# Kangfei/NNGP-src

Hardware: AMD Instinct MI355X
Metric: NNGP kernel-build + GP-solve wall-clock (ms) and GFLOP/s at N train queries (higher is better)
Workload: dtype f32 (Cholesky products as split f16 x3, f32 accumulate; f64 build/CG/means; the posterior's float64-grade residual as exact int8 digit-plane products); 1 GPU; synthetic N=32768, d=128, 5-layer ReLU NNGP + full Cholesky posterior (configs[2], north-star target); N=32768, d=128, n_relu=3, get=nngp, M_test=1024, parallelism=single GPU

## Files before the change

__graft_entry__.py:

```python
import os
import subprocess
import sys

ROOT = os.path.dirname(os.path.abspath(__file__))
for _p in (ROOT, os.path.join(ROOT, "oracle")):
    if _p not in sys.path:
        sys.path.insert(0, _p)


def build() -> None:
    env = dict(os.environ)
    env.setdefault("HIPCC", "/opt/rocm/bin/hipcc")
    subprocess.check_call(["make", "-C", os.path.join(ROOT, "nngp-src_amd", "csrc"), "-j8", "ARCH=gfx950"], env=env)
    subprocess.check_call(["make", "-C", os.path.join(ROOT, "oracle")])
    import nngp_src_amd
    from nngp_src_amd import _lib
    lib = _lib.load()
    assert lib.nngp_version() == 1
    for name in _lib.ABI_SYMBOLS + _lib.GP_ABI_SYMBOLS + _lib.ACT_ABI_SYMBOLS + _lib.MLL_ABI_SYMBOLS + _lib.LOO_ABI_SYMBOLS + _lib.ARD_ABI_SYMBOLS + _lib.ADDITIVE_ABI_SYMBOLS + _lib.POOL_ABI_SYMBOLS + _lib.SPARSE_ABI_SYMBOLS + _lib.SPARSE_EVIDENCE_ABI_SYMBOLS + _lib.I8S_ABI_SYMBOLS + _lib.MATFREE_ABI_SYMBOLS:
        assert hasattr(lib, name), name


def smoke() -> None:
    import numpy as np
    import torch
    assert torch.cuda.is_available(), "smoke() needs cuda:0"
    torch.cuda.set_device(0)
    import nngp_oracle as oracle
    from nngp_src_amd import stax, predict, batch, synth

    x, y = synth.synthetic_queries(640, 64, seed=0)
    xt, _ = synth.synthetic_queries(96, 64, seed=1)
    _, _, kernel_fn = stax.serial(stax.Dense(512), stax.Relu(), stax.Dense(1))
    kernel_fn = batch(kernel_fn, device_count=0, batch_size=0)
    predict_fn = predict.gradient_descent_mse_ensemble(kernel_fn, x, y, diag_reg=1e-3)
    mean, cov = predict_fn(x_test=xt, get="nngp", compute_cov=True)
    ref_mean, ref_cov = oracle.Posterior(x, y, oracle.make_arch(1), diag_reg=1e-3).predict(xt, "nngp", True)
    rel = np.linalg.norm(mean - ref_mean) / np.linalg.norm(ref_mean)
    assert rel < 1e-6, "posterior mean differs from the float64 oracle: %g" % rel
    assert np.allclose(np.diag(cov), np.diag(ref_cov), rtol=1e-3), "posterior variance differs from the oracle"
    info = predict_fn.model_for("nngp").info()
    print("smoke ok: mean rel-l2 %.2e, cg iters %d, rel residual %.1e" % (rel, info["refine_iters"], info["rel_residual"]))


if __name__ == "__main__":
    build()
    if len(sys.argv) > 1 and sys.argv[1] == "smoke":
        smoke()
```

nngp-src_amd/_lib.py:

```python
from __future__ import annotations

import ctypes
import os

import numpy as np

_HERE = os.path.dirname(os.path.abspath(__file__))
LIB_PATH = os.path.join(_HERE, "libnngp_hip.so")
KNOBS_LIB_PATH = os.path.join(_HERE, "libnngp_hip_knobs.so")

GET_NNGP, GET_NTK = 1, 2
DTYPE_F32, DTYPE_F64 = 0, 1
COV_NONE, COV_DIAG, COV_FULL = 0, 1, 2
MAX_DENSE = 16

ABI_SYMBOLS = (
    "nngp_version", "nngp_last_error", "nngp_kernel_build", "nngp_kernel_diag", "nngp_model_create",
    "nngp_model_destroy", "nngp_model_fit", "nngp_model_set_train", "nngp_model_build_rows",
    "nngp_model_factor", "nngp_model_factor_begin", "nngp_model_factor_panel", "nngp_model_factor_update",
    "nngp_model_factor_end", "nngp_model_factor_buffers", "nngp_model_solve", "nngp_model_append", "nngp_model_kernel_buffer", "nngp_model_info",
    "nngp_model_alpha", "nngp_model_predict", "nngp_model_set_refine", "nngp_model_cov_iters", "nngp_model_sweep_estimate", "nngp_model_factor_shift", "nngp_model_prepare_serving", "nngp_potrf_f32", "nngp_gemm_nt_f32",
    "nngp_gemm_nt_h3", "nngp_gemm_nt_f64", "nngp_trsm_rlt_f32", "nngp_model_apply_factor",
    "nngp_model_factor_input_rows", "nngp_model_factor_input_complete", "nngp_model_precond", "nngp_model_matvec_rows", "nngp_model_set_alpha", "nngp_encoder_create", "nngp_encoder_destroy", "nngp_encoder_dim",
    "nngp_encoder_encode", "nngp_comm_unique_id", "nngp_comm_create", "nngp_comm_destroy", "nngp_comm_library",
    "nngp_allgather_rows", "nngp_bcast", "nngp_model_update_timer", "nngp_model_update_timer_read", "nngp_symv_f64",
    "nngp_pool_select", "nngp_model_update_timer_bytes", "nngp_model_factor_update_cols", "nngp_gemm_nt_i8s", "nngp_model_residual_timer", "nngp_model_residual_timer_read", "nngp_model_trsm_timer", "nngp_model_trsm_timer_read", "nngp_model_residual_floor",
    "nngp_trsm_ticket_order", "nngp_trsm_ticket_queues", "nngp_model_reserve", "nngp_alloc_count",
)

GP_ABI_SYMBOLS = (
    "nngp_rbf_gp_create", "nngp_rbf_gp_destroy", "nngp_rbf_gp_set_train", "nngp_rbf_gp_evaluate", "nngp_rbf_gp_terms",
    "nngp_rbf_gp_predict", "nngp_rbf_gp_kernel", "nngp_rbf_gp_factor_buffer", "nngp_potrf_f64",
    "nngp_potrf_dinv_f64", "nngp_trsm_fwd_f64", "nngp_factor_solve_f64",
)


ACT_ABI_SYMBOLS = ("nngp_kernel_build_act", "nngp_kernel_diag_act", "nngp_model_create_act")
ACT_RELU, ACT_ABRELU, ACT_ERF = 0, 1, 2
ACTIVATIONS = {"relu": (ACT_RELU, 0), "abrelu": (ACT_ABRELU, 2), "erf": (ACT_ERF, 3)}

MLL_ABI_SYMBOLS = ("nngp_mll_create", "nngp_mll_destroy", "nngp_mll_set_train", "nngp_mll_evaluate", "nngp_mll_terms",
                   "nngp_mll_factor_buffer")


LOO_ABI_SYMBOLS = ("nngp_mll_loo_evaluate", "nngp_mll_loo_predictions", "nngp_mll_loo_terms")
LOO_NLPD, LOO_MSE = 0, 1

ARD_ABI_SYMBOLS = ("nngp_mll_reserve_ard", "nngp_mll_evaluate_ard", "nngp_mll_loo_evaluate_ard", "nngp_mll_ard_terms")

ADDITIVE_ABI_SYMBOLS = ("nngp_kernel_build_additive", "nngp_kernel_diag_additive", "nngp_model_create_additive")
MAX_GROUPS = 1024

ADDITIVE_MLL_ABI_SYMBOLS = ("nngp_mll_reserve_additive", "nngp_mll_evaluate_additive", "nngp_mll_additive_terms")

POOL_ABI_SYMBOLS = ("nngp_pool_select_greedy",)

SPARSE_ABI_SYMBOLS = ("nngp_sparse_create", "nngp_sparse_destroy", "nngp_sparse_set_inducing", "nngp_sparse_add_rows",
                      "nngp_sparse_finish", "nngp_sparse_predict", "nngp_sparse_info", "nngp_syrk_tn_f64")

SPARSE_EVIDENCE_ABI_SYMBOLS = ("nngp_sparse_reserve_evidence", "nngp_sparse_set_kernel", "nngp_sparse_evidence",
                               "nngp_sparse_evidence_grad", "nngp_sparse_evidence_terms", "nngp_sparse_adjoint_rect")
SPARSE_ARD_ABI_SYMBOLS = ("nngp_sparse_reserve_ard", "nngp_sparse_set_relevance", "nngp_sparse_evidence_grad_ard",
                          "nngp_sparse_ard_terms", "nngp_sparse_ard_rect")
I8S_ABI_SYMBOLS = ("nngp_i8s_cut_rows", "nngp_i8s_cut_sym", "nngp_i8s_residual")
MATFREE_ABI_SYMBOLS = ("nngp_matfree_create", "nngp_matfree_destroy", "nngp_matfree_fit", "nngp_matfree_solve",
                       "nngp_matfree_predict", "nngp_matfree_alpha", "nngp_matfree_info", "nngp_kmv_f64")
BOUND_DTC, BOUND_VFE = 0, 1
BOUNDS = {"dtc": BOUND_DTC, "vfe": BOUND_VFE}


class NngpArch(ctypes.Structure):
    _fields_ = [("n_dense", ctypes.c_int32), ("reserved", ctypes.c_int32),
                ("w_std", ctypes.c_double * MAX_DENSE), ("b_std", ctypes.c_double * MAX_DENSE)]


class NngpArchAct(ctypes.Structure):
    _fields_ = [("base", NngpArch), ("act", ctypes.c_int32 * (MAX_DENSE - 1)),
                ("p", (ctypes.c_double * 3) * (MAX_DENSE - 1))]


class NngpGroups(ctypes.Structure):
    _fields_ = [("n_groups", ctypes.c_int32), ("reserved", ctypes.c_int32),
                ("begin", ctypes.POINTER(ctypes.c_int32)), ("end", ctypes.POINTER(ctypes.c_int32)),
                ("weight", ctypes.POINTER(ctypes.c_double)), ("full_weight", ctypes.c_double)]


class NngpFitInfo(ctypes.Structure):
    _fields_ = [("reg", ctypes.c_double), ("trace_mean", ctypes.c_double), ("rel_residual", ctypes.c_double),
                ("refine_iters", ctypes.c_int32), ("clamped_pivots", ctypes.c_int32),
                ("n", ctypes.c_int64), ("n_padded", ctypes.c_int64)]


class NngpSparseInfo(ctypes.Structure):
    _fields_ = [("n", ctypes.c_int64), ("m", ctypes.c_int64), ("m_padded", ctypes.c_int64), ("chunks", ctypes.c_int64),
                ("sigma2", ctypes.c_double), ("trace_mean", ctypes.c_double), ("jitter_added", ctypes.c_double)]


class NngpMatfreeInfo(ctypes.Structure):
    _fields_ = [("n", ctypes.c_int64), ("m", ctypes.c_int64), ("sigma2", ctypes.c_double), ("iterations", ctypes.c_int32),
                ("k_passes", ctypes.c_int32), ("rel_residual", ctypes.c_double), ("converged", ctypes.c_int32),
                ("restarts", ctypes.c_int32)]


class NngpError(RuntimeError):
    pass


_libs = {}


def load(knobs: bool = False):
    knobs = bool(knobs) or os.environ.get("NNGP_KNOBS", "0") == "1"
    if knobs in _libs:
        return _libs[knobs]
    path = KNOBS_LIB_PATH if knobs else LIB_PATH
    if not os.path.exists(path):
        raise NngpError(
            "%s is missing (%s). Build it with `python -c 'import __graft_entry__ as g; g.build()'` "
            "or `make -C nngp-src_amd/csrc`; there is no CPU fallback." % (os.path.basename(path), path))
    import torch
    lib = ctypes.CDLL(path)
    bind_prototypes(lib, knobs)
    bind_gp_prototypes(lib)
    bind_act_prototypes(lib)
    bind_mll_prototypes(lib)
    bind_loo_prototypes(lib)
    bind_ard_prototypes(lib)
    bind_additive_prototypes(lib)
    bind_additive_mll_prototypes(lib)
    bind_pool_prototypes(lib)
    bind_sparse_prototypes(lib)
    bind_sparse_evidence_prototypes(lib)
    bind_sparse_ard_prototypes(lib)
    bind_i8s_prototypes(lib)
    bind_matfree_prototypes(lib)
    _libs[knobs] = lib
    return lib


def bind_prototypes(lib, knobs: bool = False):
    vp, i64, i32, dbl = ctypes.c_void_p, ctypes.c_int64, ctypes.c_int32, ctypes.c_double
    archp = ctypes.POINTER(NngpArch)
    lib.nngp_version.restype = ctypes.c_int
    lib.nngp_last_error.restype = ctypes.c_char_p
    if knobs:
        lib.nngp_debug_set.argtypes = [i32, i32]
        lib.nngp_debug_set.restype = ctypes.c_int
    lib.nngp_kernel_build.argtypes = [vp, i64, vp, i64, i32, archp, i32, vp, vp, i64, i64, i64, vp]
    lib.nngp_kernel_diag.argtypes = [vp, i64, i32, archp, vp, vp, vp]
    lib.nngp_model_create.argtypes = [ctypes.POINTER(vp), i64, i64, i32, i32, archp, i32, dbl, i32]
    lib.nngp_model_destroy.argtypes = [vp]
    lib.nngp_model_fit.argtypes = [vp, vp, vp, i64, vp]
    lib.nngp_model_set_train.argtypes = [vp, vp, vp, i64, vp]
    lib.nngp_model_build_rows.argtypes = [vp, i64, i64, vp]
    lib.nngp_model_factor.argtypes = [vp, vp]
    lib.nngp_model_factor_begin.argtypes = [vp, vp]
    lib.nngp_model_factor_panel.argtypes = [vp, i64, i64, vp]
    lib.nngp_model_factor_update.argtypes = [vp, i64, i64, i64, i64, vp]
    lib.nngp_model_factor_end.argtypes = [vp, vp]
    lib.nngp_model_factor_buffers.argtypes = [vp, ctypes.POINTER(vp), ctypes.POINTER(i64), ctypes.POINTER(vp)]
    lib.nngp_model_solve.argtypes = [vp, i32, dbl, vp]
    lib.nngp_model_kernel_buffer.argtypes = [vp, ctypes.POINTER(vp), ctypes.POINTER(i64)]
    lib.nngp_model_info.argtypes = [vp, ctypes.POINTER(NngpFitInfo)]
    lib.nngp_model_alpha.argtypes = [vp, vp, vp]
    lib.nngp_model_predict.argtypes = [vp, vp, i64, i32, vp, vp, vp]
    lib.nngp_encoder_create.argtypes = [ctypes.POINTER(vp), ctypes.c_char_p, i32, i32]
    lib.nngp_encoder_destroy.argtypes = [vp]
    lib.nngp_encoder_dim.argtypes = [vp]
    lib.nngp_encoder_encode.argtypes = [vp, ctypes.c_char_p, i64, i32, vp, vp, i64, ctypes.POINTER(i64)]
    lib.nngp_model_set_refine.argtypes = [vp, i32]
    lib.nngp_model_cov_iters.argtypes = [vp]
    lib.nngp_model_prepare_serving.argtypes = [vp, vp]
    lib.nngp_model_factor_shift.argtypes = [vp]
    lib.nngp_model_factor_shift.restype = ctypes.c_double
    lib.nngp_model_cov_iters.restype = ctypes.c_int
    lib.nngp_model_sweep_estimate.argtypes = [vp, ctypes.POINTER(dbl), ctypes.POINTER(dbl)]
    lib.nngp_model_append.argtypes = [vp, vp, vp, i64, vp]
    lib.nngp_gemm_nt_f64.argtypes = [vp, i64, vp, i64, vp, i64, vp, i64, i64, i64, i64, dbl, dbl, vp]
    lib.nngp_gemm_nt_i8s.argtypes = [vp, i64, vp, i64, vp, i64, vp, i64, i64, i64, i64, dbl, dbl, i32, i32, i32, vp]
    lib.nngp_potrf_f32.argtypes = [vp, i64, i64, vp, vp, vp]
    lib.nngp_gemm_nt_f32.argtypes = [vp, i64, vp, i64, vp, i64, i64, i64, i64, ctypes.c_float, ctypes.c_float, i32, vp]
    lib.nngp_gemm_nt_h3.argtypes = [vp, i64, vp, i64, vp, i64, i64, i64, i64, ctypes.c_float, ctypes.c_float,
                                    ctypes.c_float, i32, vp]
    lib.nngp_trsm_rlt_f32.argtypes = [vp, i64, i64, vp, i64, vp, i64, vp]
    lib.nngp_model_apply_factor.argtypes = [vp, vp, i64, i32, vp]
    lib.nngp_model_factor_input_rows.argtypes = [vp, i64, i64, ctypes.c_double, vp]
    lib.nngp_model_factor_input_complete.argtypes = [vp]
    lib.nngp_model_precond.argtypes = [vp, vp, vp, vp]
    lib.nngp_model_matvec_rows.argtypes = [vp, vp, vp, i64, i64, vp]
# ... 319 lines not shown
```

nngp-src_amd/csrc/api.hip:

```cpp
#include "model.h"

namespace nngp {

static thread_local char g_err[1024] = "";

void set_error(const char* fmt, ...) {
    va_list ap;
    va_start(ap, fmt);
    vsnprintf(g_err, sizeof(g_err), fmt, ap);
    va_end(ap);
}

int make_arch_dev(const nngp_arch* arch, ArchDev* out) {
    NNGP_REQUIRE(arch != nullptr, "arch is NULL");
    NNGP_REQUIRE(arch->n_dense >= 1 && arch->n_dense <= NNGP_MAX_DENSE, "arch.n_dense must be in [1, %d] (got %d)",
                 NNGP_MAX_DENSE, arch->n_dense);
    out->n_dense = arch->n_dense;
    out->groups = nullptr;
    for (int l = 0; l < NNGP_MAX_DENSE; ++l) {
        out->w2[l] = l < arch->n_dense ? arch->w_std[l] * arch->w_std[l] : 0.0;
        out->b2[l] = l < arch->n_dense ? arch->b_std[l] * arch->b_std[l] : 0.0;
    }
    return 0;
}
// ... 261 lines not shown
        rc = groups_create(groups, d, &m->groups, &plain);
        if (rc != 0) {
            delete m;
            return rc;
        }
        if (!plain) m->arch.groups = &m->groups;
    }
    m->n_cap = n_cap; m->np_cap = round_up(n_cap, TB); m->m_cap = 0;
    m->ld = m->np_cap;
    m->d = d; m->ny = ny; m->get = get; m->diag_reg = diag_reg; m->absolute = diag_reg_absolute_scale;
    const int64_t np = m->np_cap;
    auto A = [&](int r) { if (rc == 0) rc = r; };
    A(dev_alloc(&m->x, n_cap * d)); A(dev_alloc(&m->y, n_cap * ny)); A(dev_alloc(&m->q, n_cap));
    A(dev_alloc(&m->kdiag, n_cap)); A(dev_alloc(&m->k64, np * np)); A(dev_alloc(&m->a32, np * np));
    A(dev_alloc(&m->dinv, (np / TB) * TB * TB)); A(dev_alloc(&m->clamped, 1)); A(dev_alloc(&m->alpha, n_cap * ny));
    A(dev_alloc(&m->pcg.r, np)); A(dev_alloc(&m->pcg.z, np)); A(dev_alloc(&m->pcg.p, np)); A(dev_alloc(&m->pcg.q, np));
    A(dev_alloc(&m->pcg.xcol, np)); A(dev_alloc(&m->pcg.bcol, np));
    A(dev_alloc(&m->pcg.f32a, np)); A(dev_alloc(&m->pcg.f32b, np)); A(dev_alloc(&m->pcg.f32c, np));
    A(dev_alloc(&m->pcg.scal, 32));
    A(dev_alloc(&m->pcg.symv_part, (np / TB) * np));
    A(dev_alloc(&m->pcg.dot_part, 32));
    A(dev_alloc(&m->pcg.dot_ctr, 1));
    if (rc == 0 && hipMemset(m->pcg.dot_ctr, 0, sizeof(unsigned)) != hipSuccess) rc = -1;
    m->pcg.symv_np = np;
    {
        const int64_t bs_cap = triinv_block(np);
        const int64_t nblk = (np + bs_cap - 1) / bs_cap;
        A(dev_alloc(&m->tri.tinv, nblk * bs_cap * bs_cap)); A(dev_alloc(&m->tri.xinv, nblk * bs_cap * bs_cap));
        A(dev_alloc(&m->tri.partial, (bs_cap / TB) * np)); A(dev_alloc(&m->tri.tmp, bs_cap));
    }
    if (rc == 0 && hipHostMalloc(reinterpret_cast<void**>(&m->pcg.host_scal), sizeof(double) * 32) != hipSuccess) {
        set_error("model_create: hipHostMalloc failed");
        rc = -1;
    }
    if (rc == 0) rc = lookahead_create(&m->la);
    int prio_least = 0, prio_greatest = 0;
    if (hipDeviceGetStreamPriorityRange(&prio_least, &prio_greatest) != hipSuccess) prio_least = prio_greatest = 0;
    if (rc == 0 && (hipStreamCreateWithPriority(&m->solve_stream, hipStreamNonBlocking, prio_greatest) != hipSuccess ||
                    hipEventCreateWithFlags(&m->alpha_solve.ev_ready, hipEventDisableTiming) != hipSuccess ||
                    hipEventCreateWithFlags(&m->ev_lt, hipEventDisableTiming) != hipSuccess ||
                    hipEventCreateWithFlags(&m->alpha_solve.ev_solved, hipEventDisableTiming) != hipSuccess ||
                    hipEventCreateWithFlags(&m->alpha_solve.ev_predict, hipEventDisableTiming) != hipSuccess)) {
        set_error("model_create: could not create the solve stream");
        rc = -1;
    }
    if (rc == 0 && np >= 4 * kLookAheadNb) {
        m->split.rows_cap = np + 256;
        m->split.k_cap = kLookAheadNb;
        m->split.col_stride = m->split.rows_cap * m->split.k_cap * 4;
        const int64_t ncols = (np + kLookAheadNb - 1) / kLookAheadNb;
        rc = dev_alloc(&m->split.planes, ncols * m->split.col_stride);
        if (rc == 0) rc = dev_alloc(&m->split.counters, 16);
        if (rc == 0 && hipMemset(m->split.counters, 0, 16 * sizeof(int)) != hipSuccess) rc = -1;
        if (rc == 0 && !soft_alloc(&m->split.planes_t, ncols * m->split.col_stride)) m->split.planes_t = nullptr;
        if (rc == 0) rc = dev_alloc(&m->split.ldiag, 2 * kLookAheadNb * kLookAheadNb * 4);
        if (rc == 0) rc = dev_alloc(&m->split.dfrag, 2 * kLookAheadNb * 128);
        if (rc == 0) rc = dev_alloc(&m->split.dscale, 2 * kLookAheadNb);
    }
    if (rc == 0 && m_cap > 0) rc = ensure_predict_capacity(m, m_cap, true);
    if (rc != 0) {
        delete m;
        return rc;
    }
    *out = m;
    return 0;
}

int64_t nngp_alloc_count(void) { return (int64_t)g_alloc_count.load(std::memory_order_relaxed); }

int nngp_model_reserve(nngp_model* m, int64_t rows, int32_t cov_mode) {
    NNGP_REQUIRE(m != nullptr && rows > 0 && cov_mode >= NNGP_COV_NONE && cov_mode <= NNGP_COV_FULL, "reserve: bad arguments");
    NNGP_TRY(ensure_predict_capacity(m, rows, true));
    if (cov_mode == NNGP_COV_NONE) return 0;
    const int64_t mp = round_up(rows, TB);
    if (m->var_refine >= 1 || m->get == NNGP_GET_NTK) NNGP_TRY(ensure_refine_capacity(m, mp));
    const bool split_path = m->split.planes != nullptr && mp <= m->split.mb_cap && mp >= 256 && mp * m->np_cap >= 7000000;
    if (!split_path) NNGP_TRY(ensure_lt_alloc(m));
    NNGP_TRY(i8s_reserve(m, mp, cov_mode));
    if (cov_mode == NNGP_COV_FULL) NNGP_TRY(ensure_full_cov_capacity(m, rows));
    return 0;
}

int nngp_model_destroy(nngp_model* m) {
    if (m) {
        (void)hipDeviceSynchronize();
        delete m;
    }
    return 0;
}

int nngp_model_set_train(nngp_model* m, const double* x, const double* y, int64_t n, void* stream) {
    hipStream_t s = (hipStream_t)stream;
    NNGP_REQUIRE(m != nullptr && x != nullptr && y != nullptr, "set_train: NULL argument");
    NNGP_REQUIRE(n > 0 && n <= m->n_cap, "set_train: n=%lld outside (0, n_cap=%lld]", (long long)n, (long long)m->n_cap);
    m->alpha_solve.plan.invalidate();
    m->n = n;
    m->np = round_up(n, TB);
    m->built = m->factored = false;
    m->serving_ready = false;
    NNGP_HIP_CHECK(hipMemcpyAsync(m->x, x, sizeof(double) * n * m->d, hipMemcpyDeviceToDevice, s));
    NNGP_HIP_CHECK(hipMemcpyAsync(m->y, y, sizeof(double) * n * m->ny, hipMemcpyDeviceToDevice, s));
    NNGP_TRY(launch_row_sqnorm(m->x, n, m->d, m->q, s));
    NNGP_TRY(launch_kernel_diag(m->x, m->q, n, m->d, m->arch, m->get == NNGP_GET_NNGP ? m->kdiag : nullptr,
                                m->get == NNGP_GET_NTK ? m->kdiag : nullptr, s));
    hipLaunchKernelGGL(k_sum, dim3(1), dim3(1024), 0, s, m->kdiag, n, m->pcg.scal + 6);
    NNGP_HIP_CHECK(hipMemcpyAsync(m->pcg.host_scal + 6, m->pcg.scal + 6, 2 * sizeof(double), hipMemcpyDeviceToHost, s));
// ... 248 lines not shown
    return 0;
}

int nngp_model_update_timer_read(nngp_model* m, int64_t* launches, double* ms_total, double* flops_total) {
    NNGP_REQUIRE(m != nullptr && m->la != nullptr, "update_timer_read: no timer on this model");
    double ms = 0.0, fl = 0.0;
    for (int t = 0; t < m->la->tu_count; ++t) {
        NNGP_HIP_CHECK(hipEventSynchronize(m->la->tu1[t]));
        float e = 0.0f;
        NNGP_HIP_CHECK(hipEventElapsedTime(&e, m->la->tu0[t], m->la->tu1[t]));
        ms += e;
        fl += m->la->tu_flops[t];
    }
    if (launches) *launches = m->la->tu_count;
    if (ms_total) *ms_total = ms;
    if (flops_total) *flops_total = fl;
    return 0;
}

int nngp_model_residual_timer(nngp_model* m, int32_t enable) {
    NNGP_REQUIRE(m != nullptr, "residual_timer: NULL model");
    return i8s_timer_enable(m, enable);
}

int nngp_model_residual_timer_read(nngp_model* m, int64_t* launches, double* ms_total, double* flops_total, double* int8_ops_total) {
    NNGP_REQUIRE(m != nullptr, "residual_timer_read: NULL model");
    return i8s_timer_read(m, launches, ms_total, flops_total, int8_ops_total);
}

int nngp_model_trsm_timer(nngp_model* m, int32_t enable) {
    NNGP_REQUIRE(m != nullptr, "trsm_timer: NULL model");
    m->trsm_t.enable(enable != 0);
    return 0;
}

int nngp_model_trsm_timer_read(nngp_model* m, int64_t* solves, double* ms_total, double* flops_total) {
    NNGP_REQUIRE(m != nullptr, "trsm_timer_read: NULL model");
    auto& w = m->trsm_t;
    double ms = 0.0, fl = 0.0;
    NNGP_TRY(w.read(&ms));
    for (int t = 0; t < w.count; ++t) fl += m->trsm_flops[t];
    if (solves) *solves = w.count;
    if (ms_total) *ms_total = ms;
    if (flops_total) *flops_total = fl;
    w.count = 0;
    return 0;
}

int nngp_model_residual_floor(nngp_model* m, double* ratio, int32_t* distrusted) {
    NNGP_REQUIRE(m != nullptr, "residual_floor: NULL model");
    return i8s_residual_floor(m, ratio, distrusted);
}

int nngp_model_update_timer_bytes(nngp_model* m, double* bytes_total) {
    NNGP_REQUIRE(m != nullptr && m->la != nullptr && bytes_total != nullptr, "update_timer_bytes: no timer on this model");
    double b = 0.0;
    for (int t = 0; t < m->la->tu_count; ++t) b += m->la->tu_bytes[t];
    *bytes_total = b;
    return 0;
}

int nngp_model_info(nngp_model* m, nngp_fit_info* info) {
    NNGP_REQUIRE(m != nullptr && info != nullptr, "model_info: NULL argument");
    NNGP_TRY(tickets_check(m, true));
    NNGP_TRY(run_pending_solve(m, nullptr, false));
    int32_t cl = 0;
    if (m->factored) NNGP_HIP_CHECK(hipMemcpy(&cl, m->clamped, sizeof(int32_t), hipMemcpyDeviceToHost));
    info->reg = m->reg;
    info->trace_mean = m->trace_mean;
    info->rel_residual = m->alpha_solve.plan.relres;
    info->refine_iters = m->alpha_solve.plan.iters;
    info->clamped_pivots = cl;
    info->n = m->n;
    info->n_padded = m->np;
    return 0;
}

int nngp_model_cov_iters(nngp_model* m) {
    NNGP_REQUIRE(m != nullptr, "cov_iters: NULL model");
    return m->cov_iters;
}

int nngp_model_sweep_estimate(nngp_model* m, double* row_rel, double* var_rel) {
    NNGP_REQUIRE(m != nullptr, "sweep_estimate: NULL model");
    if (row_rel) *row_rel = m->sweep_est;
    if (var_rel) *var_rel = m->sweep_est_var;
    return 0;
}

int nngp_model_set_refine(nngp_model* m, int32_t sweeps) {
    NNGP_REQUIRE(m != nullptr && sweeps >= 0 && sweeps <= 8, "set_refine: level must be in [0, 8]");
    m->var_refine = sweeps;
    return 0;
}

}
```

nngp-src_amd/csrc/api_ops.hip:

```cpp
#include "model.h"
#include "gp_f64.h"
#include "trsm_order.h"
#include "../../include/nngp_i8s.h"

extern "C" {

int nngp_trsm_ticket_order(int32_t row_tiles, int32_t block_cols, int32_t tail_tiles, int32_t backward, int32_t workers, int32_t merged,
                           int32_t* items, int64_t cap, int64_t* count) {
    return tk_order_export(row_tiles, block_cols, tail_tiles, backward, workers, merged, 1, items, nullptr, cap, count);
}

int nngp_trsm_ticket_queues(int32_t row_tiles, int32_t block_cols, int32_t tail_tiles, int32_t backward, int32_t workers, int32_t merged,
                            int32_t queues, int32_t* items, int32_t* queue_of, int64_t cap, int64_t* count) {
    return tk_order_export(row_tiles, block_cols, tail_tiles, backward, workers, merged, queues, items, queue_of, cap, count);
}

int nngp_potrf_f32(float* a, int64_t n, int64_t ld, float* dinv, int32_t* clamped, void* stream) {
    NNGP_REQUIRE(a != nullptr && dinv != nullptr, "potrf_f32: NULL argument");
    if (clamped) NNGP_HIP_CHECK(hipMemsetAsync(clamped, 0, sizeof(int32_t), (hipStream_t)stream));
    return potrf_f32(a, n, ld, dinv, clamped, 0.0f, (hipStream_t)stream);
}

int nngp_potrf_f64(double* a, int64_t n, int64_t ld, void* stream) {
    hipStream_t s = (hipStream_t)stream;
    NNGP_REQUIRE(a != nullptr && n > 0 && n % TB == 0, "potrf_f64: n must be a positive multiple of %d (n=%lld)", TB, (long long)n);
    double* dinv = nullptr;
    int* status = nullptr;
    NNGP_HIP_CHECK(hipMallocAsync(reinterpret_cast<void**>(&dinv), sizeof(double) * (size_t)n * TB, s));
    NNGP_HIP_CHECK(hipMallocAsync(reinterpret_cast<void**>(&status), sizeof(int), s));
    int rc = potrf_f64(a, n, ld, dinv, status, s);
    if (rc == 0) rc = potrf_f64_status(status, s, "potrf_f64");
    (void)hipFreeAsync(dinv, s);
    (void)hipFreeAsync(status, s);
    return rc;
}

int nngp_potrf_dinv_f64(double* a, int64_t n, int64_t ld, double* dinv, void* stream) {
    hipStream_t s = (hipStream_t)stream;
    NNGP_REQUIRE(a != nullptr && dinv != nullptr && n > 0 && n % TB == 0, "potrf_dinv_f64: n must be a positive multiple of %d (n=%lld)", TB,
                 (long long)n);
    NNGP_REQUIRE(((uintptr_t)dinv & 15) == 0, "potrf_dinv_f64: dinv must be 16-byte aligned");
    int* status = nullptr;
    NNGP_HIP_CHECK(hipMallocAsync(reinterpret_cast<void**>(&status), sizeof(int), s));
    int rc = potrf_f64(a, n, ld, dinv, status, s);
    if (rc == 0) rc = potrf_f64_status(status, s, "potrf_dinv_f64");
    (void)hipFreeAsync(status, s);
    return rc;
}

int nngp_trsm_fwd_f64(double* bt, int64_t ldb, int64_t rows, const double* l, int64_t ldl, const double* dinv, int64_t n, int32_t tri,
                      void* stream) {
    hipStream_t s = (hipStream_t)stream;
    NNGP_REQUIRE(bt != nullptr && l != nullptr && dinv != nullptr, "trsm_fwd_f64: NULL argument");
    NNGP_REQUIRE(rows > 0 && n > 0 && rows % TB == 0 && n % TB == 0, "trsm_fwd_f64: rows, n must be positive multiples of %d (rows=%lld n=%lld)",
                 TB, (long long)rows, (long long)n);
    NNGP_REQUIRE(tri == 0 || rows == n, "trsm_fwd_f64: the triangular mode solves the identity, rows must equal n (rows=%lld n=%lld)",
                 (long long)rows, (long long)n);
    NNGP_REQUIRE(ldb >= n && ldl >= n && ldb % 2 == 0 && ldl % 2 == 0, "trsm_fwd_f64: ldb, ldl must be >= n and even (ldb=%lld ldl=%lld n=%lld)",
                 (long long)ldb, (long long)ldl, (long long)n);
    NNGP_REQUIRE((((uintptr_t)bt | (uintptr_t)l | (uintptr_t)dinv) & 15) == 0, "trsm_fwd_f64: operands must be 16-byte aligned");
    double* t = nullptr;
    NNGP_HIP_CHECK(hipMallocAsync(reinterpret_cast<void**>(&t), sizeof(double) * (size_t)rows * TB, s));
    const int rc = trsm_fwd_f64(bt, ldb, rows, l, ldl, dinv, n, t, tri != 0, s);
    (void)hipFreeAsync(t, s);
    return rc;
}

// ... 36 lines not shown

int nngp_gemm_nt_f32(float* c, int64_t ldc, const float* a, int64_t lda, const float* b, int64_t ldb, int64_t m,
                     int64_t n, int64_t k, float alpha, float beta, int32_t lower_only, void* stream) {
    NNGP_REQUIRE(a != nullptr && b != nullptr && c != nullptr, "gemm_nt_f32: NULL argument");
    return launch_gemm_nt_f32(c, ldc, a, lda, b, ldb, m, n, k, alpha, beta, lower_only != 0, (hipStream_t)stream);
}

namespace {
struct H3Scratch {
    hipStream_t stream = nullptr;
    char* p = nullptr;
    size_t bytes = 0;
    bool used = false;
};
std::mutex g_h3_scratch_mutex;
H3Scratch g_h3_scratch[4];

int h3_scratch_get(hipStream_t s, size_t bytes, char** out) {
    std::lock_guard<std::mutex> lock(g_h3_scratch_mutex);
    H3Scratch* e = nullptr;
    for (auto& c : g_h3_scratch)
        if (c.used && c.stream == s) e = &c;
    if (e == nullptr)
        for (auto& c : g_h3_scratch)
            if (!c.used && e == nullptr) e = &c;
    if (e == nullptr) {
        e = &g_h3_scratch[0];
        if (hipStreamSynchronize(e->stream) != hipSuccess) {
            (void)hipGetLastError();
            NNGP_HIP_CHECK(hipDeviceSynchronize());
        }
        (void)hipFree(e->p);
        *e = H3Scratch();
    }
    if (e->bytes < bytes) {
        if (e->p != nullptr) {
            NNGP_HIP_CHECK(hipStreamSynchronize(s));
            (void)hipFree(e->p);
            e->p = nullptr;
            e->bytes = 0;
        }
        NNGP_HIP_CHECK(hipMalloc((void**)&e->p, bytes));
        e->bytes = bytes;
    }
    e->used = true;
    e->stream = s;
    *out = e->p;
    return 0;
}
}

int nngp_gemm_nt_h3(float* c, int64_t ldc, const float* a, int64_t lda, const float* b, int64_t ldb, int64_t m, int64_t n,
                    int64_t k, float alpha, float beta, float scale, int32_t lower_only, void* stream) {
    hipStream_t s = (hipStream_t)stream;
    NNGP_REQUIRE(a != nullptr && b != nullptr && c != nullptr && scale > 0.0f, "gemm_nt_h3: bad argument");
    NNGP_REQUIRE(m > 0 && n > 0 && k > 0 && k % 32 == 0, "gemm_nt_h3: k must be a multiple of 32");
    const int64_t mp = round_up(m, 256), np = round_up(n, 256), ldp = 4 * k;
    char* pa = nullptr;
    NNGP_TRY(h3_scratch_get(s, (size_t)((mp + np) * ldp + 64), &pa));
    char* pb = pa + mp * ldp;
    int* counters = reinterpret_cast<int*>(pb + np * ldp);
    if (mp > m) NNGP_HIP_CHECK(hipMemsetAsync(pa + m * ldp, 0, (size_t)((mp - m) * ldp), s));
    NNGP_HIP_CHECK(hipMemsetAsync(pb + n * ldp, 0, (size_t)((np - n) * ldp + 64), s));
    NNGP_TRY(launch_split_rows(a, lda, m, k, scale, pa, ldp, s));
    NNGP_TRY(launch_split_rows(b, ldb, n, k, scale, pb, ldp, s));
    return launch_gemm_nt_h3(c, ldc, pa, pb, ldp, m, n, k, alpha / (scale * scale), beta, lower_only != 0, 0, counters,
                             NNGP_KNOB(4) > 0 ? NNGP_KNOB(4) : 0, s);
}

int nngp_gemm_nt_f64(double* c, int64_t ldc, const double* cin, int64_t ldcin, const double* a, int64_t lda,
                     const double* b, int64_t ldb, int64_t m, int64_t n, int64_t k, double alpha, double beta,
                     void* stream) {
    NNGP_REQUIRE(a != nullptr && b != nullptr && c != nullptr, "gemm_nt_f64: NULL argument");
    return launch_gemm_nt_f64(c, ldc, cin, ldcin, a, lda, b, ldb, m, n, k, alpha, beta, (hipStream_t)stream);
}

int nngp_gemm_nt_i8s(double* c, int64_t ldc, const double* cin, int64_t ldcin, const double* a, int64_t lda, const double* b,
                     int64_t ldb, int64_t m, int64_t n, int64_t k, double alpha, double beta, int32_t slices_a, int32_t slices_b,
                     int32_t cut, void* stream) {
    hipStream_t s = (hipStream_t)stream;
    NNGP_REQUIRE(a != nullptr && b != nullptr && c != nullptr && m > 0 && n > 0 && k > 0 && m % TB == 0 && n % TB == 0 && ldc >= n &&
                     lda >= k && ldb >= k,
                 "gemm_nt_i8s: m, n must be multiples of %d", TB);
    I8Plan pl;
    NNGP_TRY(i8s_plan(slices_a, slices_b, cut, &pl));
    const int64_t mp = round_up(m, 256), np = round_up(n, 256), kp = round_up(k, 128);
    const int64_t nchunk = i8s_chunks(k, &pl);
    const int64_t slab = m * n;
    const size_t plane_bytes = (size_t)((mp * slices_a + np * slices_b) * kp);
    const size_t part_bytes = (size_t)(nchunk * pl.ndiag * slab) * sizeof(int32_t);
    NNGP_REQUIRE(part_bytes < (size_t)16 << 30, "gemm_nt_i8s: the test entry keeps all partial products (16 GB limit)");
    char* ws = nullptr;
    NNGP_HIP_CHECK(hipMalloc((void**)&ws, plane_bytes + part_bytes + sizeof(double) * (size_t)(m + n) + 64));
    NNGP_HIP_CHECK(hipMemsetAsync(ws, 0, plane_bytes, s));
    int8_t* pa = reinterpret_cast<int8_t*>(ws);
    int8_t* pb = pa + mp * slices_a * kp;
    int32_t* part = reinterpret_cast<int32_t*>(ws + plane_bytes);
    double* sca = reinterpret_cast<double*>(ws + plane_bytes + part_bytes);
    double* scb = sca + m;
    int* counters = reinterpret_cast<int*>(scb + n);
    NNGP_HIP_CHECK(hipMemsetAsync(counters, 0, 64, s));
    int rc = launch_i8s_slice_rows(a, lda, m, k, slices_a, nullptr, sca, pa, kp, mp * kp, s);
    if (rc == 0) rc = launch_i8s_slice_rows(b, ldb, n, k, slices_b, nullptr, scb, pb, kp, np * kp, s);
    if (rc == 0)
        rc = launch_gemm_nt_i8s(part, n, slab, pa, kp, mp * kp, pb, kp, np * kp, pl, m, n, k, counters,
                                NNGP_KNOB(4) > 0 ? NNGP_KNOB(4) : 0, s);
    if (rc == 0)
        rc = launch_i8s_combine(c, ldc, cin ? cin : c, cin ? ldcin : ldc, beta, alpha, nullptr, 0, 0.0, part, n, slab, (int)nchunk,
                                pl.ndiag, sca, scb, m, n, s);
    (void)hipStreamSynchronize(s);
    (void)hipFree(ws);
    return rc;
}

int nngp_i8s_cut_rows(const double* src, int64_t ld, int64_t rows, int64_t cols, int32_t ns, const double* scale_in, double* scale_out,
                      int8_t* planes, int64_t ldp, double* writeback, void* stream) {
    NNGP_REQUIRE(src != nullptr && planes != nullptr && (scale_in != nullptr || scale_out != nullptr), "i8s_cut_rows: NULL argument");
    NNGP_REQUIRE(ns >= 2 && ns <= 7, "i8s_cut_rows: 2..7 planes (ns=%d)", (int)ns);
    NNGP_REQUIRE(rows > 0 && cols > 0 && ld >= cols && ld % 2 == 0, "i8s_cut_rows: ld must be even and >= cols (rows=%lld cols=%lld ld=%lld)",
                 (long long)rows, (long long)cols, (long long)ld);
// ... 180 lines not shown
```

nngp-src_amd/csrc/common.h:

```cpp
#pragma once
#include <hip/hip_runtime.h>
#include <stdint.h>
#include <atomic>
#include <stdio.h>
#include <string.h>

#include "../../include/nngp_hip.h"
#include "../../include/nngp_rbf_gp.h"
#include "../../include/nngp_activations.h"
#include "../../include/nngp_mll.h"
#include "../../include/nngp_additive.h"
#include "../../include/nngp_pool.h"
#include "../../include/nngp_sparse.h"

namespace nngp {

constexpr int TB = 128;

void set_error(const char* fmt, ...);
void note_alloc();
#ifdef NNGP_TIMING_KNOBS
extern std::atomic<int> g_knobs[16];
#define NNGP_KNOB(i) (nngp::g_knobs[i].load(std::memory_order_relaxed))
#else
// ... 54 lines not shown
    int64_t n1, n2;
    int d;
    int64_t row_begin, row_end;
    int sym;
    double* nngp64;
    double* ntk64;
    float* nngp32;
    float* ntk32;
    int64_t ld64, ld32;
    double diag_add_nngp32;
    double diag_add_ntk32;
    int lower32;
    const double* comp;
    int no_comp;
};
inline BuildArgs symmetric_build_args(const double* x, const double* q, int64_t n, int d) {
    BuildArgs a{};
    a.x1 = a.x2 = x;
    a.q1 = a.q2 = q;
    a.n1 = a.n2 = n;
    a.d = d;
    a.row_begin = 0;
    a.row_end = n;
    a.sym = 1;
    return a;
}
int launch_row_sqnorm(const double* x, int64_t n, int d, double* q, hipStream_t s);
int launch_diag_from_q(const double* q, int64_t n, const ArchDev& arch, double* dn, double* dt, hipStream_t s);
int launch_kernel_build(const BuildArgs& a, const ArchDev& arch, hipStream_t s);
int launch_kernel_build_plain(const BuildArgs& a, const ArchDev& arch, hipStream_t s);
int plan_build_tiles(const BuildArgs& a, bool rows_at_4, int64_t* tiles_r, int64_t* tiles_c, int64_t* nblocks, int* vec_ok);
int launch_kernel_diag(const double* x, const double* q, int64_t n, int d, const ArchDev& arch, double* dn, double* dt,
                       hipStream_t s);

int groups_create(const nngp_groups* g, int d, GroupsDev* out, bool* plain);
void groups_destroy(GroupsDev* g);
int launch_kernel_build_additive(const BuildArgs& a, const ArchDev& arch, hipStream_t s);
int launch_diag_additive(const double* x, const double* q, int64_t n, int d, const ArchDev& arch, double* dn, double* dt,
                         hipStream_t s);

int launch_gemm_nt_f32(float* c, int64_t ldc, const float* a, int64_t lda, const float* b, int64_t ldb,
                       int64_t m, int64_t n, int64_t k, float alpha, float beta, bool lower_only, hipStream_t s, int tri = 0);

int launch_gemm_nt_f32_batched(float* c, int64_t ldc, const float* a, int64_t lda, const float* b, int64_t ldb,
                               int64_t m, int64_t n, int64_t k, float alpha, float beta, bool lower_only, int batch,
                               int64_t stride_c, int64_t stride_a, int64_t stride_b, hipStream_t s, int tri = 0);

int launch_split_rows(const float* p, int64_t ld, int64_t rows, int64_t k, float scale, char* out, int64_t out_ld,
                      hipStream_t s);
int launch_split_rows_rowscale(const float* src, int64_t ld_src, int64_t rows, int64_t k, float* copy_dst, int64_t ld_copy,
                               char* out, int64_t out_ld, float* row_inv, hipStream_t s, int64_t pan_stride = 0);
int launch_split_lower_t(const float* l, int64_t ld, int64_t n, int64_t bs, float scale, char* out, int64_t col_stride,
                         hipStream_t s);
int launch_gemm_nt_h3(float* c, int64_t ldc, const char* a, const char* b, int64_t ldp, int64_t m, int64_t n, int64_t k,
                      float alpha, float beta, bool lower_only, int64_t diag_shift, int* counters, int reserve_cus,
                      hipStream_t s, const float* row_alpha = nullptr);
struct H3RegionSpec {
    int64_t row0, col0, m, n, shift;
};
int launch_gemm_nt_h3r(float* c, int64_t ldc, const char* a, const char* b, int64_t ldp, int64_t pstride, int npanels, int64_t lead,
                       const H3RegionSpec* spec, int nreg, int64_t k, float alpha, float beta, bool lower_only, int* counters,
                       int reserve_cus, hipStream_t s, const float* row_alpha = nullptr, int helper = 0);
int launch_gemm_nt_h3x(float* c, int64_t ldc, const char* a, const char* b, int64_t ldp, int64_t pstride, int npanels, int64_t lead,
                       int64_t m, int64_t n, int64_t k, float alpha, float beta, bool lower_only, int64_t diag_shift, int* counters,
                       int reserve_cus, hipStream_t s, const float* row_alpha = nullptr);

int launch_potrf_leaf(float* a, int64_t ld, float* dinv_block, int32_t* clamped, float pivot_floor, hipStream_t s);
int potrf_f32(float* a, int64_t n, int64_t ld, float* dinv, int32_t* clamped, float pivot_floor, hipStream_t s);
int potrf_rec(float* a, int64_t n, int64_t ld, float* dinv, int32_t* clamped, float pivot_floor, hipStream_t s);
int trsm_rlt_f32(float* b, int64_t ldb, int64_t m, const float* l, int64_t ldl, const float* dinv, int64_t n,
                 hipStream_t s);
int trsm_rut_f32(float* b, int64_t ldb, int64_t m, const float* lt, int64_t ldl, const float* dinvt, int64_t n,
                 hipStream_t s);

int launch_trsm_panel_f32(float* b, int64_t ldb, int64_t m, const float* l, int64_t ldl, const float* dinv, int64_t w,
                          char* planes, int64_t ldp, float scale, hipStream_t s, char* planes_t = nullptr, int64_t tstride = 0,
                          int64_t row0 = 0, int64_t col0 = 0);
int launch_split_diag_frag(const float* a, int64_t ld, int64_t w, float scale, char* out, const float* dinv, float* dfrag,
                           float* dscale, hipStream_t s);
int launch_trsm_panel_h3(float* b, int64_t ldb, int64_t m, const char* lfrag, const float* dfrag, const float* dscale, int64_t w,
                         char* planes, int64_t ldp, float scale, hipStream_t s, char* planes_t = nullptr, int64_t tstride = 0,
                         int64_t row0 = 0, int64_t col0 = 0);


struct SplitWork {
    char* planes = nullptr;
    int64_t rows_cap = 0, k_cap = 0, col_stride = 0;
    float scale = 1.0f;
    int* counters = nullptr;
    bool l_ready = false;
    int64_t split_panel = -1;
    char* ldiag = nullptr;
    float* dfrag = nullptr;
    float* dscale = nullptr;
    char* planes_t = nullptr;
    bool lt_ready = false;
    char* planes_b = nullptr;
    int b_panels = 1;
    int solve_reserve = 0;
    float* row_inv = nullptr;
    int64_t mb_cap = 0;
};

struct LookAhead {
    static constexpr int kMaxSteps = 64;
    hipStream_t panel = nullptr, update = nullptr;
    hipStream_t bulk = nullptr;
    hipStream_t aux = nullptr;
    hipStream_t side = nullptr;
    hipEvent_t ev_side_done = nullptr;
    int prio_levels = 0;
    bool masked = false;
    hipEvent_t ev_in = nullptr, ev_panel_done = nullptr, ev_update_done = nullptr;
    hipEvent_t ev_panel[kMaxSteps] = {}, ev_col[kMaxSteps] = {};
    hipEvent_t ev_chunk[kMaxSteps] = {}, ev_helper[kMaxSteps] = {};
    hipEvent_t ev_far[kMaxSteps] = {}, ev_near[kMaxSteps] = {}, ev_tc[kMaxSteps] = {}, ev_tb[kMaxSteps] = {}, ev_split[kMaxSteps] = {},
               ev_gp[kMaxSteps] = {};
    hipEvent_t ev_c1[kMaxSteps] = {};
    hipEvent_t ev_chain[kMaxSteps] = {};
    hipEvent_t ev_bulk_done = nullptr;
    static constexpr int kMaxTimed = 320;
    bool time_updates = false;
    hipEvent_t tu0[kMaxTimed] = {}, tu1[kMaxTimed] = {};
    int tu_count = 0;
    double tu_flops[kMaxTimed] = {};
    double tu_bytes[kMaxTimed] = {};
};
int lookahead_create(LookAhead** out);
void lookahead_destroy(LookAhead* la);
struct TriInv;
int potrf_lookahead_f32(float* a, int64_t n, int64_t ld, float* dinv, int32_t* clamped, float pivot_floor,
                        LookAhead* la, SplitWork* sw, hipStream_t user, TriInv* ti = nullptr);
constexpr int64_t kLookAheadNb = 1024;
constexpr int kLookAheadGroup = 4;
int potrf_panel_f32(float* a, int64_t n, int64_t ld, float* dinv, int32_t* clamped, float pivot_floor, int64_t o,
                    int64_t w, hipStream_t s, SplitWork* sw = nullptr);
int potrf_update_f32(float* a, int64_t n, int64_t ld, int64_t po, int64_t pw, int64_t o, int64_t w, hipStream_t s,
                     SplitWork* sw = nullptr);
int potrf_update_cols_f32(float* a, int64_t n, int64_t ld, int64_t po, int64_t pw, const int64_t* cols, int ncols, int64_t w,
                          hipStream_t s, SplitWork* sw = nullptr);

struct I8Plan {
    int ndiag, npairs;
    int dstart[9];
    int pa[32], pb[32];
};
struct I8Planes {
    int8_t* planes = nullptr;
    double* scale = nullptr;
    bool ready = false;
    int ns_done = 0;
    int alloc_planes = 0;
};
struct I8Work {
    I8Planes k, aux;
    int64_t k_rows = 0;
    int8_t* zplanes = nullptr;
    double* zscale = nullptr;
    int64_t z_rows = 0;
    int z_planes = 0;
    int32_t* partial = nullptr;
    double* rowpart = nullptr;
    int64_t rowpart_rows = 0;
    int* counters = nullptr;
    int ns_k = 5, ns_z = 5, cut = 4;
    static constexpr int kMaxTimed = 64;
    double t_ops[kMaxTimed] = {};
    double t_flops[kMaxTimed] = {};
};
int i8s_plan(int nsa, int nsb, int cut, I8Plan* pl);
int64_t i8s_chunks(int64_t k, const I8Plan* pl = nullptr);
int launch_i8s_diag_bound_scale(const double* src, int64_t ld, int64_t n, double* scale, hipStream_t s);
int launch_i8s_scale_sqsum(const double* scale, int64_t n, double* out, hipStream_t s);
int launch_i8s_floor_ratio(const double* z, int64_t ld, int64_t rows, int64_t cols, const double* var, const I8Plan& pl, int nsa, int nsb,
                           const double* sk2, unsigned long long* out, hipStream_t s);
int launch_i8s_floor_ratio_rows(const double* zstat, int64_t rows, const double* var, const I8Plan& pl, int nsa, int nsb, const double* sk2,
                                unsigned long long* out, hipStream_t s);
int launch_i8s_slice_rows(const double* src, int64_t ld, int64_t rows, int64_t cols, int ns, const double* scale_in, double* scale_out,
                          int8_t* planes, int64_t ldp, int64_t pstride, hipStream_t s, double* writeback = nullptr);
// ... 144 lines not shown
```

nngp-src_amd/csrc/gemm_h3.hip:

```cpp
#include <atomic>

#include "common.h"

namespace nngp {

namespace {

typedef _Float16 h8 __attribute__((ext_vector_type(8)));
typedef float f32x16 __attribute__((ext_vector_type(16)));
typedef float f32x4 __attribute__((ext_vector_type(4)));
typedef unsigned int u32x4 __attribute__((ext_vector_type(4)));

constexpr int HT = 256;
constexpr int HROW = 128;
constexpr int HSTAGE = 2 * HT * HROW;

__device__ __forceinline__ int lds_off(int row, int ch) { return row * HROW + ((ch ^ ((row >> 1) & 7)) << 4); }

__global__ __launch_bounds__(256) void k_split_rows(const float* __restrict__ p, int64_t ld, int64_t rows, int k8_per_row,
                                                    float scale, char* __restrict__ out, int64_t out_ld) {
    const int64_t idx = (int64_t)blockIdx.x * 256 + threadIdx.x;
    const int64_t r = idx / k8_per_row;
    const int c8 = (int)(idx % k8_per_row);
    if (r >= rows) return;
    const f32x4* src = reinterpret_cast<const f32x4*>(p + r * ld + (int64_t)c8 * 8);
    const f32x4 v0 = src[0], v1 = src[1];
    h8 hi, lo;
#pragma unroll
    for (int e = 0; e < 8; ++e) {
        const float a = (e < 4 ? v0[e] : v1[e - 4]) * scale;
        const _Float16 h = (_Float16)a;
        hi[e] = h;
        lo[e] = (_Float16)(a - (float)h);
    }
    char* dst = out + r * out_ld + (int64_t)(c8 >> 2) * 128 + (c8 & 3) * 16;
    *reinterpret_cast<h8*>(dst) = hi;
    *reinterpret_cast<h8*>(dst + 64) = lo;
}

template <int NV>
__global__ __launch_bounds__(256) void k_split_rows_rowscale(const float* __restrict__ src, int64_t ld_src, int64_t rows,
                                                             int k, float* __restrict__ copy_dst, int64_t ld_copy,
                                                             char* __restrict__ out, int64_t out_ld, int64_t pan_stride,
                                                             float* __restrict__ row_inv) {
    const int lane = threadIdx.x & 63;
    const int64_t r = (int64_t)blockIdx.x * 4 + (threadIdx.x >> 6);
    if (r >= rows) return;
    const float* p = src + r * ld_src;
    f32x4 v[NV];
    float mx = 0.0f;
#pragma unroll
    for (int i = 0; i < NV; ++i) {
        const int k0 = 4 * (lane + 64 * i);
        v[i] = (k0 < k) ? *reinterpret_cast<const f32x4*>(p + k0) : f32x4{0.0f, 0.0f, 0.0f, 0.0f};
#pragma unroll
// ... 6 lines not shown
    const float sc = (mx > 0.0f && mx < 3.0e38f) ? ldexpf(1.0f, 14 - e2) : 1.0f;
    if (lane == 0) row_inv[r] = 1.0f / sc;
    char* o = out + r * out_ld;
#pragma unroll
    for (int i = 0; i < NV; ++i) {
        const int k0 = 4 * (lane + 64 * i);
        if (k0 >= k) continue;
        if (copy_dst != nullptr) *reinterpret_cast<f32x4*>(copy_dst + r * ld_copy + k0) = v[i];
        typedef _Float16 h4 __attribute__((ext_vector_type(4)));
        h4 hi, lo;
#pragma unroll
        for (int e = 0; e < 4; ++e) {
            const float a = v[i][e] * sc;
            const _Float16 h = (_Float16)a;
            hi[e] = h;
            lo[e] = (_Float16)(a - (float)h);
        }
        const int kp = k0 & 1023;
        char* dst = o + (int64_t)(k0 >> 10) * pan_stride + (int64_t)(kp >> 5) * 128 + (kp & 31) * 2;
        *reinterpret_cast<h4*>(dst) = hi;
        *reinterpret_cast<h4*>(dst + 64) = lo;
    }
}

__global__ __launch_bounds__(256) void k_split_lower_t(const float* __restrict__ l, int64_t ld, int64_t n, int64_t bs,
                                                       float scale, char* __restrict__ out, int64_t col_stride) {
    __shared__ float tile[32][33];
    const int64_t gk0 = (int64_t)blockIdx.y * 32;
    const int64_t r0 = (int64_t)blockIdx.x * 32;
    const int64_t j = gk0 / bs, o = j * bs;
    if (r0 >= o) return;
    const int tx = threadIdx.x & 31, ty = threadIdx.x >> 5;
#pragma unroll
    for (int i = 0; i < 4; ++i) tile[ty + 8 * i][tx] = l[(gk0 + ty + 8 * i) * ld + r0 + tx];
    __syncthreads();
    if (threadIdx.x < 128) {
        const int rr = threadIdx.x >> 2, g = threadIdx.x & 3;
        h8 hi, lo;
#pragma unroll
        for (int e = 0; e < 8; ++e) {
            const float a = tile[g * 8 + e][rr] * scale;
            const _Float16 h = (_Float16)a;
            hi[e] = h;
            lo[e] = (_Float16)(a - (float)h);
        }
        char* dst = out + j * col_stride + (r0 + rr) * (bs * 4) + ((gk0 - o) >> 5) * 128 + g * 16;
        *reinterpret_cast<h8*>(dst) = hi;
        *reinterpret_cast<h8*>(dst + 64) = lo;
    }
}

typedef __attribute__((address_space(3))) void lds_void;
typedef const __attribute__((address_space(1))) void glb_void;

__host__ __device__ __forceinline__ int h3_block_cols(int gr, int br, int bc, int tiles_m, int tiles_n, bool lower, int sh_t) {
    int last = tiles_n - 1;
    if (lower) {
        int rmax = gr * br + br - 1;
        if (rmax > tiles_m - 1) rmax = tiles_m - 1;
        if (rmax + sh_t < last) last = rmax + sh_t;
    }
    return last / bc + 1;
}

template <bool LOWER>
__global__ __launch_bounds__(512) void k_gemm_nt_h3(float* C, int64_t ldc, const char* A, const char* B, int64_t ldp,
                                                    int m, int n, int tiles_m, int nk, float alpha, float beta,
                                                    int diag_shift, int order_br, int order_bc, int* counters,
                                                    int slots_per_xcd, int ablate, const float* row_alpha) {
    __shared__ __attribute__((aligned(1024))) char smem[2 * HSTAGE + 16];
    int& s_slot = *reinterpret_cast<int*>(smem + 2 * HSTAGE);
    const int tid = threadIdx.x;
    const int lane = tid & 63, wave = tid >> 6;
    const int wr = wave >> 2, wc = wave & 3;
    const int tiles_n = (n + HT - 1) / HT;
    const int xcd = blockIdx.x & 7;
    const int group = __builtin_amdgcn_readfirstlane(wr);
    const int w4 = __builtin_amdgcn_readfirstlane(wc);
    const int l3 = lane >> 3;
    const int frow = lane & 31, fh = lane >> 5;
    const int64_t lane_off = (int64_t)l3 * ldp + (((lane & 7) ^ ((4 * (w4 & 1) + (l3 >> 1)) & 7)) << 4);

    for (;;) {
        if (tid == 0) s_slot = atomicAdd(&counters[xcd], 1);
        __syncthreads();
        const int slot = s_slot;
        __syncthreads();
        if (slot >= slots_per_xcd) {
            if (tid == 0 && atomicAdd(&counters[8], 1) == (int)gridDim.x - 1)
                for (int i = 0; i < 9; ++i) __hip_atomic_store(&counters[i], 0, __ATOMIC_RELAXED, __HIP_MEMORY_SCOPE_AGENT);
            break;
        }
        int bi, bj;
        {
            const int per = order_br * order_bc;
            int G = (slot / per) * 8 + xcd;
            const int i = slot % per;
            const int brows = (tiles_m + order_br - 1) / order_br;
            const int sh_t = (diag_shift + HT - 1) / HT;
            int gr = 0;
            for (; gr < brows; ++gr) {
                const int cnt = h3_block_cols(gr, order_br, order_bc, tiles_m, tiles_n, LOWER, sh_t);
                if (G < cnt) break;
                G -= cnt;
            }
            if (gr >= brows) continue;
            bi = gr * order_br + (i % order_br);
            bj = G * order_bc + (i / order_br);
            if (bi >= tiles_m || bj >= tiles_n) continue;
        }
        if (LOWER && bj * HT > bi * HT + HT - 1 + diag_shift) continue;

        const char* Ab = A + (int64_t)bi * HT * ldp;
        const char* Bb = B + (int64_t)bj * HT * ldp;
        auto glds_stage = [&](int t, int buf) {
            const int64_t koff = (int64_t)(nk - 1 - t) * 128 + lane_off;
// ... 75 lines not shown
                __builtin_amdgcn_s_setprio(0);
                __builtin_amdgcn_sched_barrier(0);
                if (kk == 0) asm volatile("s_waitcnt vmcnt(0)" ::: "memory");
                __builtin_amdgcn_s_barrier();
                __builtin_amdgcn_sched_barrier(0);
            }
        }
        if (group == 0) __builtin_amdgcn_s_barrier();

        const int row_base = bi * HT + group * 128;
        const int col_base = bj * HT + w4 * 64;
#pragma unroll
        for (int i = 0; i < 4; ++i) {
            float cold[2][16], ra[16];
            bool live[2];
            if (row_alpha != nullptr) {
                const int rr = row_base + i * 32 + 4 * fh;
#pragma unroll
                for (int r = 0; r < 16; ++r) ra[r] = (rr < m) ? row_alpha[rr + (r & 3) + 8 * (r >> 2)] : 1.0f;
            }
#pragma unroll
            for (int j = 0; j < 2; ++j) {
                const int r0 = row_base + i * 32, c0 = col_base + j * 32;
                live[j] = r0 < m && c0 < n && !(LOWER && (c0 >> 7) > ((r0 + diag_shift) >> 7)) && !(ablate & 8);
                if (live[j] && beta != 0.0f) {
                    const float* p0 = C + (int64_t)(r0 + 4 * fh) * ldc + c0 + frow;
#pragma unroll
                    for (int r = 0; r < 16; ++r) cold[j][r] = p0[(int64_t)((r & 3) + 8 * (r >> 2)) * ldc];
                }
            }
#pragma unroll
            for (int j = 0; j < 2; ++j) {
                if (!live[j]) {
                    asm volatile("" ::"v"(acc[i][j]));
                    continue;
                }
                const int r0 = row_base + i * 32, c0 = col_base + j * 32;
                float* p0 = C + (int64_t)(r0 + 4 * fh) * ldc + c0 + frow;
#pragma unroll
                for (int r = 0; r < 16; ++r) {
                    float v = alpha * acc[i][j][r];
                    if (row_alpha != nullptr) v *= ra[r];
                    if (beta != 0.0f) v = fmaf(beta, cold[j][r], v);
                    p0[(int64_t)((r & 3) + 8 * (r >> 2)) * ldc] = v;
                }
            }
        }
    }
}


typedef float f32x4v __attribute__((ext_vector_type(4)));

struct H3Region {
    int64_t c_off;
    int64_t a_off;
    int64_t b_off;
    int m, n, shift, blk0;
};
struct H3Regions {
    int count, nblk;
    H3Region r[4];
};

#ifdef NNGP_TIMING_KNOBS
__device__ unsigned long long g_h3_stamps[2 * 8];
#endif
template <bool LOWER, int ABL>
__global__ __launch_bounds__(512) void k_gemm_nt_h3v2(float* C, int64_t ldc, const char* A, const char* B, int64_t ldp,
                                                      int64_t pstride, int npanels, int nk_first, int first_off, H3Regions regs, int nk,
                                                      float alpha, float beta, int order_br, int order_bc,
                                                      int* counters, int slots_per_xcd, const float* row_alpha, int total_wgs) {
    constexpr int ablate = ABL;
    __shared__ __attribute__((aligned(1024))) char smem[8 * 20480];
    int& s_slot = *reinterpret_cast<int*>(smem);
    const int tid = threadIdx.x;
    const int lane = tid & 63, wave = tid >> 6;
    const int xcd = blockIdx.x & 7;
    const int group = __builtin_amdgcn_readfirstlane(wave >> 2);
    const int w4 = __builtin_amdgcn_readfirstlane(wave & 3);
    const int l3 = lane >> 3;
    const int r16 = lane & 15, q4 = lane >> 4;
    const unsigned lane_off = (unsigned)l3 * (unsigned)ldp + (((lane & 7) ^ ((4 * (w4 & 1) + (l3 >> 1)) & 7)) << 4);
    const unsigned frag_hi = (unsigned)r16 * HROW + (((unsigned)q4 ^ ((unsigned)r16 >> 1)) << 4);
    const unsigned frag_lo = frag_hi ^ 64u;
    const int nstage = (npanels - 1) * nk + nk_first;

    int vx = xcd, tries = 0;
    struct Tile {
        const char* pa;
        const char* pb;
        float* pc;
        int row0, col0;
        int m, n, shift;
    };
    auto decode = [&](int slot, Tile& tl) -> bool {
        const int per = order_br * order_bc;
        int G = (slot / per) * 8 + vx;
        const int i = slot % per;
        if (G >= regs.nblk) return false;
        int ri = 0;
#pragma unroll
        for (int r = 1; r < 4; ++r)
            if (r < regs.count && G >= regs.r[r].blk0) ri = r;
        const int m = regs.r[ri].m, n = regs.r[ri].n, diag_shift = regs.r[ri].shift;
        G -= regs.r[ri].blk0;
        const int tiles_m = (m + HT - 1) / HT, tiles_n = (n + HT - 1) / HT;
        const int brows = (tiles_m + order_br - 1) / order_br;
        const int sh_t = (diag_shift + HT - 1) / HT;
        int gr = 0;
        for (; gr < brows; ++gr) {
            const int cnt = h3_block_cols(gr, order_br, order_bc, tiles_m, tiles_n, LOWER, sh_t);
            if (G < cnt) break;
            G -= cnt;
        }
        if (gr >= brows) return false;
        const int bi = gr * order_br + (i % order_br);
        const int bj = G * order_bc + (i / order_br);
        if (bi >= tiles_m || bj >= tiles_n) return false;
        if (LOWER && bj * HT > bi * HT + HT - 1 + diag_shift) return false;
        tl.pa = A + regs.r[ri].a_off + (int64_t)bi * HT * ldp;
        tl.pb = B + regs.r[ri].b_off + (int64_t)bj * HT * ldp;
        tl.pc = C + regs.r[ri].c_off + (int64_t)bi * HT * ldc + (int64_t)bj * HT;
        tl.row0 = bi * HT;
        tl.col0 = bj * HT;
        tl.m = m;
        tl.n = n;
        tl.shift = diag_shift;
        return true;
    };
    int cur_p = 0, cur_kb = 0;
    auto cursor_reset = [&]() { cur_p = 0; cur_kb = (npanels == 1 ? nk_first : nk) - 1; };
    auto cursor_take = [&]() -> int64_t {
        const int64_t off = (int64_t)cur_kb * 128 - (int64_t)cur_p * pstride + (cur_p == npanels - 1 ? first_off : 0);
        if (--cur_kb < 0) {
            ++cur_p;
            cur_kb = (cur_p == npanels - 1 ? nk_first : nk) - 1;
        }
        return off;
    };
    auto glds_b = [&](int t, int64_t koff, const char* tile_pb) {
        const char* pb = tile_pb + koff;
        char* dst = smem + (t & 1) * HSTAGE + HT * HROW;
#pragma unroll
        for (int e = 0; e < 4; ++e) {
            const int piece = group * 16 + e * 4 + w4;
            __builtin_amdgcn_global_load_lds((glb_void*)(pb + (int64_t)piece * 8 * ldp + lane_off), (lds_void*)(dst + piece * 1024), 16, 0, 0);
        }
    };
    auto glds_a = [&](int t, int64_t koff, const char* tile_pa) {
        const char* pa = tile_pa + koff;
        char* dst = smem + (t & 1) * HSTAGE;
#pragma unroll
        for (int e = 0; e < 4; ++e) {
            const int piece = group * 16 + e * 4 + w4;
            __builtin_amdgcn_global_load_lds((glb_void*)(pa + (int64_t)piece * 8 * ldp + lane_off), (lds_void*)(dst + piece * 1024), 16, 0, 0);
        }
    };
    auto fetch_tile = [&](Tile& tl) -> bool {
        for (;;) {
            if (tid == 0) s_slot = atomicAdd(&counters[vx], 1);
            __syncthreads();
            const int slot = __builtin_amdgcn_readfirstlane(s_slot);
            __syncthreads();
            if (slot >= slots_per_xcd) {
                if (++tries >= 8) return false;
                vx = (vx + 1) & 7;
                continue;
            }
            if (decode(slot, tl)) return true;
        }
    };

#ifdef NNGP_TIMING_KNOBS
    const bool stamping = (ablate & 256) && blockIdx.x == 0 && (wave == 0 || wave == 4) && lane == 0;
    unsigned long long st_last = 0, st_k0 = 0, st_r0 = 0;
    if (stamping) { st_k0 = __builtin_amdgcn_s_memtime(); st_r0 = __builtin_amdgcn_s_memrealtime(); }
#define H3_STAMP(i) do { if (stamping) { const unsigned long long now_ = __builtin_amdgcn_s_memtime(); \
                         if ((i) >= 0) g_h3_stamps[(wave >> 2) * 8 + ((i) < 0 ? 0 : (i))] += now_ - st_last; st_last = now_; } } while (0)
#else
#define H3_STAMP(i) do { } while (0)
#endif
    Tile tl = {};
    bool have = fetch_tile(tl);
    if (have) {
        cursor_reset();
        const int64_t k0 = cursor_take();
        glds_b(0, k0, tl.pb);
        glds_a(0, k0, tl.pa);
    }
    while (have) {
        f32x4v acc[8][4];
#pragma unroll
        for (int i = 0; i < 8; ++i)
#pragma unroll
            for (int j = 0; j < 4; ++j) acc[i][j] = f32x4v{0.0f, 0.0f, 0.0f, 0.0f};

        asm volatile("s_waitcnt vmcnt(0)" ::: "memory");
        __builtin_amdgcn_s_barrier();
        if (group == 1) __builtin_amdgcn_s_barrier();
        H3_STAMP(st_last == 0 ? -1 : 4);
        int next_slot = 0;
        for (int t = 0; t < nstage; ++t) {
            const char* sa_ = smem + (t & 1) * HSTAGE;
            const char* sb_ = sa_ + HT * HROW;
            const bool more = t + 1 < nstage && !(ablate & 1);
            const int64_t knext = more ? cursor_take() : 0;
            h8 bh[4], bl[4], ah[4], al[4];
#pragma unroll
            for (int j = 0; j < 4; ++j) {
                const int rb = (w4 * 64 + j * 16) * HROW;
                bh[j] = *reinterpret_cast<const h8*>(sb_ + rb + frag_hi);
                bl[j] = *reinterpret_cast<const h8*>(sb_ + rb + frag_lo);
            }
#pragma unroll
            for (int i = 0; i < 4; ++i) {
                const int rb = (group * 128 + i * 16) * HROW;
                ah[i] = *reinterpret_cast<const h8*>(sa_ + rb + frag_hi);
                al[i] = *reinterpret_cast<const h8*>(sa_ + rb + frag_lo);
            }
            if (more) {
                glds_b(t + 1, knext, tl.pb);
                if (t > 0) asm volatile("s_waitcnt vmcnt(4)" ::: "memory");
            } else {
                asm volatile("s_waitcnt vmcnt(0)" ::: "memory");
                if (tid == 0) next_slot = atomicAdd(&counters[vx], 1);
            }
            asm volatile("s_waitcnt lgkmcnt(0)" ::: "memory");
            __builtin_amdgcn_sched_barrier(0);
            __builtin_amdgcn_s_barrier();
            __builtin_amdgcn_sched_barrier(0);
            __builtin_amdgcn_s_setprio(1);
            if (!(ablate & 2)) {
#pragma unroll
                for (int i = 0; i < 4; ++i)
#pragma unroll
                    for (int j = 0; j < 4; ++j) acc[i][j] = __builtin_amdgcn_mfma_f32_16x16x32_f16(bl[j], ah[i], acc[i][j], 0, 0, 0);
#pragma unroll
                for (int i = 0; i < 4; ++i)
#pragma unroll
                    for (int j = 0; j < 4; ++j) acc[i][j] = __builtin_amdgcn_mfma_f32_16x16x32_f16(bh[j], al[i], acc[i][j], 0, 0, 0);
#pragma unroll
                for (int i = 0; i < 4; ++i)
#pragma unroll
                    for (int j = 0; j < 4; ++j) acc[i][j] = __builtin_amdgcn_mfma_f32_16x16x32_f16(bh[j], ah[i], acc[i][j], 0, 0, 0);
            } else {
#pragma unroll
                for (int i = 0; i < 4; ++i) asm volatile("" ::"v"(ah[i]), "v"(al[i]), "v"(bh[i]), "v"(bl[i]));
            }
            __builtin_amdgcn_s_setprio(0);
            __builtin_amdgcn_sched_barrier(0);
            __builtin_amdgcn_s_barrier();
            __builtin_amdgcn_sched_barrier(0);
#pragma unroll
            for (int i = 0; i < 4; ++i) {
                const int rb = (group * 128 + 64 + i * 16) * HROW;
                ah[i] = *reinterpret_cast<const h8*>(sa_ + rb + frag_hi);
                al[i] = *reinterpret_cast<const h8*>(sa_ + rb + frag_lo);
            }
            if (more) {
                glds_a(t + 1, knext, tl.pa);
                asm volatile("s_waitcnt vmcnt(4)" ::: "memory");
            }
            asm volatile("s_waitcnt lgkmcnt(0)" ::: "memory");
            __builtin_amdgcn_sched_barrier(0);
            __builtin_amdgcn_s_barrier();
            __builtin_amdgcn_sched_barrier(0);
            __builtin_amdgcn_s_setprio(1);
            if (!(ablate & 2)) {
#pragma unroll
                for (int i = 0; i < 4; ++i)
#pragma unroll
                    for (int j = 0; j < 4; ++j) acc[4 + i][j] = __builtin_amdgcn_mfma_f32_16x16x32_f16(bl[j], ah[i], acc[4 + i][j], 0, 0, 0);
#pragma unroll
                for (int i = 0; i < 4; ++i)
#pragma unroll
                    for (int j = 0; j < 4; ++j) acc[4 + i][j] = __builtin_amdgcn_mfma_f32_16x16x32_f16(bh[j], al[i], acc[4 + i][j], 0, 0, 0);
#pragma unroll
                for (int i = 0; i < 4; ++i)
#pragma unroll
                    for (int j = 0; j < 4; ++j) acc[4 + i][j] = __builtin_amdgcn_mfma_f32_16x16x32_f16(bh[j], ah[i], acc[4 + i][j], 0, 0, 0);
            } else {
#pragma unroll
                for (int i = 0; i < 4; ++i) asm volatile("" ::"v"(ah[i]), "v"(al[i]), "v"(bh[i]), "v"(bl[i]));
            }
            __builtin_amdgcn_s_setprio(0);
            __builtin_amdgcn_sched_barrier(0);
            if (more) asm volatile("s_waitcnt vmcnt(2)" ::: "memory");
            __builtin_amdgcn_s_barrier();
            __builtin_amdgcn_sched_barrier(0);
        }
        if (group == 0) __builtin_amdgcn_s_barrier();

        H3_STAMP(0);
        const Tile ct = tl;
        if (tid == 0) s_slot = next_slot;
        __syncthreads();
        int slot = __builtin_amdgcn_readfirstlane(s_slot);
        __syncthreads();
        have = slot < slots_per_xcd && decode(slot, tl);
        if (!have) {
            if (slot >= slots_per_xcd) {
                ++tries;
                vx = (vx + 1) & 7;
            }
            have = tries < 8 && fetch_tile(tl);
        }

        H3_STAMP(1);
        const int m = ct.m, n = ct.n, diag_shift = ct.shift;
        const int row_base = ct.row0 + group * 128;
        const int col_base = ct.col0 + w4 * 64;
        const unsigned voff = ((unsigned)r16 * (unsigned)ldc + 4u * (unsigned)q4) * 4u;
        char* cw = reinterpret_cast<char*>(ct.pc + (int64_t)(group * 128) * ldc + w4 * 64);
        const int64_t band = (int64_t)16 * ldc * 4;
        const bool full = !(ablate & 8) && beta != 0.0f && col_base + 64 <= n && row_base + 128 <= m &&
                          !(LOWER && (col_base >> 7) > ((row_base + diag_shift) >> 7));
        if (full) {
            constexpr int RB = 3;
            char* stage_c = smem + (wave * 20480);
            if (!(ablate & 16)) {
#pragma unroll
                for (int i = RB; i < 8; ++i)
#pragma unroll
                    for (int j = 0; j < 4; ++j)
                        __builtin_amdgcn_global_load_lds((glb_void*)(cw + i * band + voff + 64 * j),
                                                         (lds_void*)(stage_c + ((i - RB) * 4 + j) * 1024), 16, 0, (ablate & 64) ? 2 : 0);
            }
            f32x4v cold[RB][4];
            float ra[8];
#pragma unroll
            for (int i = 0; i < 8; ++i) ra[i] = alpha * (row_alpha != nullptr ? row_alpha[row_base + 16 * i + r16] : 1.0f);
#pragma unroll
            for (int i = 0; i < RB; ++i)
#pragma unroll
                for (int j = 0; j < 4; ++j)
                    cold[i][j] = (ablate & 16) ? f32x4v{0.0f, 0.0f, 0.0f, 0.0f}
                                                : (ablate & 64) ? __builtin_nontemporal_load(reinterpret_cast<const f32x4v*>(cw + i * band + voff + 64 * j))
                                                                : *reinterpret_cast<const f32x4v*>(cw + i * band + voff + 64 * j);
            auto fma_b = [&](int i, int slot_) {
#pragma unroll
                for (int j = 0; j < 4; ++j) {
#pragma unroll
                    for (int r = 0; r < 4; ++r) acc[i][j][r] = fmaf(beta, cold[slot_][j][r], ra[i] * acc[i][j][r]);
                    asm volatile("" : "+v"(acc[i][j]) : : "memory");
                }
            };
#pragma unroll
            for (int i = 0; i < RB; ++i) fma_b(i, i);
            asm volatile("s_waitcnt vmcnt(0)" ::: "memory");
#pragma unroll
            for (int i = RB; i < 8; ++i) {
#pragma unroll
                for (int j = 0; j < 4; ++j)
                    cold[(i - RB) % RB][j] = (ablate & 16) ? f32x4v{0.0f, 0.0f, 0.0f, 0.0f}
                                                           : *reinterpret_cast<const f32x4v*>(stage_c + ((i - RB) * 4 + j) * 1024 + lane * 16);
                fma_b(i, (i - RB) % RB);
            }
            H3_STAMP(2);
#pragma unroll
            for (int i = 0; i < 8; ++i)
#pragma unroll
                for (int j = 0; j < 4; ++j) {
                    if (ablate & 32)
                        asm volatile("" ::"v"(acc[i][j]));
                    else if (ablate & 64)
                        __builtin_nontemporal_store(acc[i][j], reinterpret_cast<f32x4v*>(cw + i * band + voff + 64 * j));
                    else
                        *reinterpret_cast<f32x4v*>(cw + i * band + voff + 64 * j) = acc[i][j];
                }
        } else {
#pragma unroll 1
            for (int i = 0; i < 8; ++i) {
                const int r0 = row_base + 16 * i;
                const bool live = col_base < n && r0 < m && !(LOWER && (col_base >> 7) > ((r0 + diag_shift) >> 7)) && !(ablate & 8);
                f32x4v v[4];
#pragma unroll
                for (int j = 0; j < 4; ++j) {
                    v[j] = acc[0][j];
#pragma unroll
                    for (int ii = 1; ii < 8; ++ii)
                        if (i == ii) v[j] = acc[ii][j];
                }
                if (!live) continue;
                const float sa = alpha * (row_alpha != nullptr ? row_alpha[r0 + r16] : 1.0f);
#pragma unroll
                for (int j = 0; j < 4; ++j) {
                    f32x4v* pc = reinterpret_cast<f32x4v*>(cw + i * band + voff + 64 * j);
                    f32x4v o = v[j];
                    if (beta != 0.0f) {
                        const f32x4v c0 = *pc;
#pragma unroll
                        for (int r = 0; r < 4; ++r) o[r] = fmaf(beta, c0[r], sa * o[r]);
                    } else {
#pragma unroll
                        for (int r = 0; r < 4; ++r) o[r] *= sa;
                    }
                    *pc = o;
                }
            }
        }
        H3_STAMP(3);
#ifdef NNGP_TIMING_KNOBS
        if (stamping) g_h3_stamps[(wave >> 2) * 8 + 5] += 1;
#endif
        if (ablate & 8) {
#pragma unroll
            for (int i = 0; i < 8; ++i)
#pragma unroll
                for (int j = 0; j < 4; ++j) asm volatile("" ::"v"(acc[i][j]));
        }
        if (have) {
            asm volatile("s_waitcnt lgkmcnt(0)" ::: "memory");
            __builtin_amdgcn_s_barrier();
            cursor_reset();
            const int64_t k0 = cursor_take();
            glds_b(0, k0, tl.pb);
            glds_a(0, k0, tl.pa);
        }
    }
#ifdef NNGP_TIMING_KNOBS
    if (stamping) {
        g_h3_stamps[(wave >> 2) * 8 + 6] += __builtin_amdgcn_s_memtime() - st_k0;
        g_h3_stamps[(wave >> 2) * 8 + 7] += __builtin_amdgcn_s_memrealtime() - st_r0;
    }
#endif
#undef H3_STAMP
    if (tid == 0 && atomicAdd(&counters[8], 1) == total_wgs - 1)
        for (int i = 0; i < 9; ++i) __hip_atomic_store(&counters[i], 0, __ATOMIC_RELAXED, __HIP_MEMORY_SCOPE_AGENT);
}

}

int launch_split_rows(const float* p, int64_t ld, int64_t rows, int64_t k, float scale, char* out, int64_t out_ld,
                      hipStream_t s) {
    if (rows <= 0) return 0;
    NNGP_REQUIRE(k > 0 && k % 32 == 0 && ld % 4 == 0 && ((uintptr_t)p & 15) == 0 && ((uintptr_t)out & 15) == 0 &&
                     out_ld >= 4 * k && out_ld % 16 == 0,
                 "split_rows: k must be a multiple of 32 and the operands 16-byte aligned");
    const int64_t total = rows * (k / 8);
    hipLaunchKernelGGL(k_split_rows, dim3((unsigned)((total + 255) / 256)), dim3(256), 0, s, p, ld, rows, (int)(k / 8),
                       scale, out, out_ld);
    NNGP_HIP_CHECK(hipGetLastError());
    return 0;
}

int launch_split_rows_rowscale(const float* src, int64_t ld_src, int64_t rows, int64_t k, float* copy_dst, int64_t ld_copy,
                               char* out, int64_t out_ld, float* row_inv, hipStream_t s, int64_t pan_stride) {
    if (rows <= 0) return 0;
    const int64_t kp = k < 1024 ? k : 1024;
    NNGP_REQUIRE(k > 0 && k <= 2048 && k % 32 == 0 && ld_src % 4 == 0 && ((uintptr_t)src & 15) == 0 && out_ld >= 4 * kp &&
                     out_ld % 16 == 0 && ((uintptr_t)out & 15) == 0 && row_inv != nullptr && (k <= 1024 || (pan_stride > 0 && pan_stride % 16 == 0)) &&
                     (copy_dst == nullptr || (ld_copy % 4 == 0 && ((uintptr_t)copy_dst & 15) == 0)),
                 "split_rows_rowscale: k must be a multiple of 32, at most 2048, operands 16-byte aligned");
    if (k <= 1024)
        hipLaunchKernelGGL((k_split_rows_rowscale<4>), dim3((unsigned)((rows + 3) / 4)), dim3(256), 0, s, src, ld_src, rows, (int)k,
                           copy_dst, ld_copy, out, out_ld, pan_stride, row_inv);
    else
        hipLaunchKernelGGL((k_split_rows_rowscale<8>), dim3((unsigned)((rows + 3) / 4)), dim3(256), 0, s, src, ld_src, rows, (int)k,
                           copy_dst, ld_copy, out, out_ld, pan_stride, row_inv);
    NNGP_HIP_CHECK(hipGetLastError());
    return 0;
}

int launch_split_lower_t(const float* l, int64_t ld, int64_t n, int64_t bs, float scale, char* out, int64_t col_stride,
                         hipStream_t s) {
    if (n <= bs) return 0;
    NNGP_REQUIRE(n % 32 == 0 && bs % 32 == 0 && bs > 0 && ((uintptr_t)out & 15) == 0 && col_stride % 16 == 0,
                 "split_lower_t: sizes must be multiples of 32");
    hipLaunchKernelGGL(k_split_lower_t, dim3((unsigned)(n / 32), (unsigned)(n / 32)), dim3(256), 0, s, l, ld, n, bs, scale,
                       out, col_stride);
    NNGP_HIP_CHECK(hipGetLastError());
    return 0;
}

constexpr int kH3DefaultForm = 2;

int launch_gemm_nt_h3r(float* c, int64_t ldc, const char* a, const char* b, int64_t ldp, int64_t pstride, int npanels, int64_t lead,
                       const H3RegionSpec* spec, int nreg, int64_t k, float alpha, float beta, bool lower_only, int* counters,
                       int reserve_cus, hipStream_t s, const float* row_alpha, int helper) {
    NNGP_REQUIRE(nreg >= 1 && nreg <= 4 && spec != nullptr, "gemm_nt_h3: 1 to 4 regions per launch");
    NNGP_REQUIRE(k > 0 && k % 32 == 0, "gemm_nt_h3: k must be a multiple of 32 (k=%lld)", (long long)k);
    NNGP_REQUIRE(ldp >= 4 * k && ldp % 16 == 0 && ((uintptr_t)a & 15) == 0 && ((uintptr_t)b & 15) == 0 && counters != nullptr,
                 "gemm_nt_h3: operands must be 16-byte aligned");
    NNGP_REQUIRE(npanels >= 1 && lead >= 0 && lead < k && lead % 32 == 0 && (npanels == 1 || (pstride > 0 && pstride % 16 == 0)) &&
                     ldc < (1LL << 26),
                 "gemm_nt_h3: bad panel layout");
    int form = (NNGP_KNOB(5) >= 41 && NNGP_KNOB(5) <= 42) ? NNGP_KNOB(5) - 40 : kH3DefaultForm;
    const bool c16 = ldc % 4 == 0 && ((uintptr_t)c & 15) == 0;
    if (npanels > 1 || lead > 0 || nreg > 1) {
        NNGP_REQUIRE(c16, "gemm_nt_h3: a multi-panel or multi-region product needs a 16-byte aligned C with ldc a multiple of 4");
        form = 2;
    } else if (!c16) {
        form = 1;
    }
    static const int kOrders[][2] = {{4, 4}, {8, 4}, {4, 8}, {2, 8}, {8, 2}, {8, 8}, {2, 16}, {2, 4}};
    const int variant = (NNGP_KNOB(5) >= 10 && NNGP_KNOB(5) < 18) ? NNGP_KNOB(5) - 10 : 0;
    const int br = kOrders[variant][0], bc = kOrders[variant][1];
    H3Regions regs = {};
    int64_t nblk = 0;
    for (int r = 0; r < nreg; ++r) {
        const H3RegionSpec& sp = spec[r];
        if (sp.m <= 0 || sp.n <= 0) continue;
        NNGP_REQUIRE(sp.m % 128 == 0 && sp.n % 128 == 0 && sp.shift % 128 == 0 && sp.shift >= 0 && sp.row0 >= 0 && sp.col0 >= 0 &&
                         sp.m < 2147483647LL && sp.n < 2147483647LL && sp.col0 + sp.n <= ldc && sp.col0 % 4 == 0,
                     "gemm_nt_h3: m, n must be multiples of 128 (m=%lld n=%lld)", (long long)sp.m, (long long)sp.n);
        H3Region& rg = regs.r[regs.count++];
        rg.c_off = sp.row0 * ldc + sp.col0;
        rg.a_off = sp.row0 * ldp;
        rg.b_off = sp.col0 * ldp;
        rg.m = (int)sp.m;
        rg.n = (int)sp.n;
        rg.shift = lower_only ? (int)sp.shift : 0;
        rg.blk0 = (int)nblk;
        const int64_t tm = (sp.m + HT - 1) / HT, tn = (sp.n + HT - 1) / HT;
        for (int64_t gr = 0; gr < (tm + br - 1) / br; ++gr)
            nblk += h3_block_cols((int)gr, br, bc, (int)tm, (int)tn, lower_only, (int)((rg.shift + HT - 1) / HT));
    }
    if (regs.count == 0) return 0;
    regs.nblk = (int)nblk;
    const int64_t slots_per_xcd = ((nblk + 7) / 8) * br * bc;
    NNGP_REQUIRE(slots_per_xcd < 2147483647LL / 8, "gemm_nt_h3: too many tiles");
    static std::atomic<int> ncu_cached{0};
    int ncu = ncu_cached.load(std::memory_order_relaxed);
    if (ncu == 0) {
        int dev = 0, count = 0;
        ncu = (hipGetDevice(&dev) == hipSuccess &&
               hipDeviceGetAttribute(&count, hipDeviceAttributeMultiprocessorCount, dev) == hipSuccess && count > 0) ? count : 256;
        ncu_cached.store(ncu, std::memory_order_relaxed);
    }
    int64_t grid = ncu - reserve_cus;
    if (grid > slots_per_xcd * 8) grid = slots_per_xcd * 8;
    grid = (grid / 8) * 8;
    if (grid < 8) grid = 8;
    int total_wgs = (int)grid;
    if (helper != 0) {
        NNGP_REQUIRE(form == 2 && reserve_cus >= 8 && reserve_cus % 8 == 0, "gemm_nt_h3: a helper grid needs form 2 and reserved compute units");
        total_wgs = (int)grid + reserve_cus;
        if (helper == 2) grid = reserve_cus;
    }
    const int ablate = NNGP_KNOB(0) & 507;
    if (form == 2) {
#define NNGP_H3V2_LAUNCH(LOW, ABL)                                                                                                  \
    hipLaunchKernelGGL((k_gemm_nt_h3v2<LOW, ABL>), dim3((unsigned)grid), dim3(512), 0, s, c, ldc, a, b, ldp, pstride, npanels,          \
                       (int)((k - lead) / 32), (int)(lead * 4), regs, (int)(k / 32), alpha, beta, br, bc, counters,                  \
                       (int)slots_per_xcd, row_alpha, total_wgs)
#ifdef NNGP_TIMING_KNOBS
        if (lower_only) {
            switch (ablate) {
                case 1: NNGP_H3V2_LAUNCH(true, 1); break;
                case 2: NNGP_H3V2_LAUNCH(true, 2); break;
                case 8: NNGP_H3V2_LAUNCH(true, 8); break;
                case 9: NNGP_H3V2_LAUNCH(true, 9); break;
                case 16: NNGP_H3V2_LAUNCH(true, 16); break;
                case 32: NNGP_H3V2_LAUNCH(true, 32); break;
                case 64: NNGP_H3V2_LAUNCH(true, 64); break;
                case 256: NNGP_H3V2_LAUNCH(true, 256); break;
                default: NNGP_H3V2_LAUNCH(true, 0); break;
            }
        } else
#else
        (void)ablate;
        if (lower_only)
            NNGP_H3V2_LAUNCH(true, 0);
        else
#endif
            NNGP_H3V2_LAUNCH(false, 0);
#undef NNGP_H3V2_LAUNCH
    } else {
        const H3Region& rg = regs.r[0];
        const int64_t tm = (rg.m + HT - 1) / HT;
        if (lower_only)
            hipLaunchKernelGGL((k_gemm_nt_h3<true>), dim3((unsigned)grid), dim3(512), 0, s, c + rg.c_off, ldc, a + rg.a_off, b + rg.b_off, ldp,
                               rg.m, rg.n, (int)tm, (int)(k / 32), alpha, beta, rg.shift, br, bc, counters, (int)slots_per_xcd, ablate & 11,
                               row_alpha);
        else
            hipLaunchKernelGGL((k_gemm_nt_h3<false>), dim3((unsigned)grid), dim3(512), 0, s, c + rg.c_off, ldc, a + rg.a_off, b + rg.b_off, ldp,
                               rg.m, rg.n, (int)tm, (int)(k / 32), alpha, beta, 0, br, bc, counters, (int)slots_per_xcd, ablate & 11, row_alpha);
    }
    NNGP_HIP_CHECK(hipGetLastError());
#ifdef NNGP_TIMING_KNOBS
    if (ablate == 256 && form == 2 && lower_only) {
        unsigned long long h[16];
        (void)hipDeviceSynchronize();
        if (hipMemcpyFromSymbol(h, HIP_SYMBOL(g_h3_stamps), sizeof(h)) == hipSuccess)
            for (int w = 0; w < 2; ++w)
                fprintf(stderr, "h3v2 stamps m=%d wave %d: tiles %llu  main %llu  slot %llu  c_in %llu  stores %llu  next0 %llu  | kernel cycles %llu  "
                                "realtime ticks %llu (clock %.3f GHz)\n", regs.r[0].m, 4 * w, h[w * 8 + 5], h[w * 8 + 0], h[w * 8 + 1], h[w * 8 + 2],
                        h[w * 8 + 3], h[w * 8 + 4], h[w * 8 + 6], h[w * 8 + 7], h[w * 8 + 7] ? 0.1 * (double)h[w * 8 + 6] / (double)h[w * 8 + 7] : 0.0);
    }
#endif
    return 0;
}

int launch_gemm_nt_h3x(float* c, int64_t ldc, const char* a, const char* b, int64_t ldp, int64_t pstride, int npanels, int64_t lead,
                       int64_t m, int64_t n, int64_t k, float alpha, float beta, bool lower_only, int64_t diag_shift, int* counters,
                       int reserve_cus, hipStream_t s, const float* row_alpha) {
    if (m <= 0 || n <= 0) return 0;
    NNGP_REQUIRE(ldc >= n && diag_shift % 128 == 0 && diag_shift >= 0, "gemm_nt_h3: bad ldc / diag_shift");
    const H3RegionSpec one = {0, 0, m, n, diag_shift};
    return launch_gemm_nt_h3r(c, ldc, a, b, ldp, pstride, npanels, lead, &one, 1, k, alpha, beta, lower_only, counters, reserve_cus, s,
                              row_alpha, 0);
}

int launch_gemm_nt_h3(float* c, int64_t ldc, const char* a, const char* b, int64_t ldp, int64_t m, int64_t n, int64_t k,
                      float alpha, float beta, bool lower_only, int64_t diag_shift, int* counters, int reserve_cus,
                      hipStream_t s, const float* row_alpha) {
    return launch_gemm_nt_h3x(c, ldc, a, b, ldp, 0, 1, 0, m, n, k, alpha, beta, lower_only, diag_shift, counters, reserve_cus, s,
                              row_alpha);
}

}
```

nngp-src_amd/csrc/model.h:

```cpp
#pragma once
#include <stdarg.h>
#include <stdlib.h>
#include <cmath>
#include <new>
#include <mutex>
#include "common.h"
#include "i8_trust.h"
#include "alpha_plan.h"
#include <atomic>

namespace nngp {
extern std::atomic<long long> g_alloc_count;

template <typename T>
inline int dev_alloc(T** p, int64_t count) {
    *p = nullptr;
    if (count <= 0) return 0;
    NNGP_HIP_CHECK(hipMalloc(reinterpret_cast<void**>(p), sizeof(T) * (size_t)count));
    g_alloc_count.fetch_add(1, std::memory_order_relaxed);
    return 0;
}

template <typename T>
inline void dev_free(T*& p) {
// ... 142 lines not shown
    float* trsm_tmp = nullptr;
    int64_t ktd_cap = 0;
    int64_t full_cap = 0;
    double* ktt64 = nullptr;
    float* vvt32 = nullptr;

    int var_refine = 1;
    float* lt32 = nullptr;
    float* dinvt = nullptr;
    bool lt_ready = false;
    int64_t refine_cap = 0;
    double* z64 = nullptr;
    double* r64 = nullptr;
    double* covp64 = nullptr;
    double* ainv64 = nullptr;
    bool serving_ready = false;
    bool serving_weak = false;
    RowsPcg rows{};
    int64_t rows_pq_cap = 0;
    int cov_iters = 0;
    double sweep_est_var = -1.0;
    double sweep_est = -1.0;
    double* kaux64 = nullptr;
    bool aux_ready = false;
    double* ktd_aux = nullptr;
    int64_t ktd_aux_cap = 0;

    I8Residual i8;
    AlphaSolve alpha_solve;

    double reg = 0.0, trace_mean = 0.0;
    double reg_fac = 0.0;
    hipStream_t solve_stream = nullptr;
    bool tri_stale = false, tri_pending = false;
    EventPairTimer<32> trsm_t;
    double trsm_flops[decltype(trsm_t)::kMax] = {};
    hipEvent_t ev_tri = nullptr, ev_tri_fork = nullptr;
    hipEvent_t ev_lt = nullptr;

    ~nngp_model() {
        dev_free(x); dev_free(y); dev_free(q); dev_free(kdiag); dev_free(k64); dev_free(a32); dev_free(dinv);
        dev_free(clamped); dev_free(alpha);
        groups_destroy(&groups);
        dev_free(pcg.r); dev_free(pcg.z); dev_free(pcg.p); dev_free(pcg.q); dev_free(pcg.xcol); dev_free(pcg.bcol);
        dev_free(pcg.f32a); dev_free(pcg.f32b); dev_free(pcg.f32c); dev_free(pcg.scal); dev_free(pcg.symv_part); dev_free(pcg.dot_part); dev_free(pcg.dot_ctr);
        if (pcg.host_scal) (void)hipHostFree(pcg.host_scal);
        if (pcg.iter_graph) (void)hipGraphExecDestroy(pcg.iter_graph);
        dev_free(tri.tinv); dev_free(tri.xinv); dev_free(tri.partial); dev_free(tri.tmp);
        lookahead_destroy(la);
        if (solve_stream) (void)hipStreamDestroy(solve_stream);
        if (ev_lt) (void)hipEventDestroy(ev_lt);
        if (ev_tri) (void)hipEventDestroy(ev_tri);
        if (ev_tri_fork) (void)hipEventDestroy(ev_tri_fork);
        dev_free(split.planes); dev_free(split.counters); dev_free(split.planes_t); dev_free(split.planes_b); dev_free(split.row_inv);
        dev_free(split.ldiag); dev_free(split.dfrag); dev_free(split.dscale);
        tk_destroy(tk);
        dev_free(xt_q); dev_free(tt_diag); dev_free(ktd64); dev_free(b32); dev_free(trsm_tmp); dev_free(ktt64); dev_free(vvt32);
        dev_free(lt32); dev_free(dinvt); dev_free(z64); dev_free(r64); dev_free(covp64); dev_free(kaux64); dev_free(ktd_aux);
        dev_free(ainv64);
        dev_free(rows.p); dev_free(rows.q); dev_free(rows.rho); dev_free(rows.coef); dev_free(rows.tol); dev_free(rows.delta);
        dev_free(rows.var); dev_free(rows.state); dev_free(rows.live); dev_free(rows.zstat);
        if (rows.host) (void)hipHostFree(rows.host);
    }
};


namespace nngp {
struct ResidualNote {
    bool want_fused_rows = false;
    bool fused = false;
    bool used_int8 = false;
};


enum class CovCheck {
    None,
    NngpDiag,
    NngpFull,
    Ntk,
    NngpDiagLevel1,
};

struct PredictCall {
    hipStream_t s = nullptr;
    const double* xt = nullptr;
    const double* qt = nullptr;
    const double* ktd = nullptr;
    const double* ktd_nngp = nullptr;
    int64_t mt = 0, mp = 0;
    bool on_train = false, is_ntk = false, want_cov = false, full = false;
    bool compact_train = false;
    bool serving = false;
    double *mean = nullptr, *var_or_cov = nullptr;
    bool z_valid = false;
    bool used_i8 = false;
    bool i8_check_pending = false;
    CovCheck check = CovCheck::None;
};

int ensure_predict_capacity(nngp_model* m, int64_t mt, bool need_ktd);
int ensure_full_cov_capacity(nngp_model* m, int64_t mt);
void set_split_scale(nngp_model* m);
int ensure_refine_capacity(nngp_model* m, int64_t mp);
int ensure_lt_alloc(nngp_model* m);
int ensure_lt(nngp_model* m, hipStream_t s);
int ensure_lt_split(nngp_model* m, hipStream_t s);
int tri_join(nngp_model* m, hipStream_t s);
// ... 36 lines not shown
```

nngp-src_amd/csrc/potrf_lookahead.hip:

```cpp
#include <cstdio>
#include <new>

#include "common.h"

namespace nngp {

int lookahead_create(LookAhead** out) {
    LookAhead* la = new (std::nothrow) LookAhead();
    NNGP_REQUIRE(la != nullptr, "lookahead_create: out of memory");
    int ncu = 256;
    hipDeviceProp_t prop;
    int dev = 0;
    if (hipGetDevice(&dev) == hipSuccess && hipGetDeviceProperties(&prop, dev) == hipSuccess) ncu = prop.multiProcessorCount;
    const int panel_cus = NNGP_KNOB(4) > 0 ? NNGP_KNOB(4) : 32;
    bool masked = false;
    if (NNGP_KNOB(5) == 2 && ncu >= 64 && panel_cus < ncu) {
        const int words = (ncu + 31) / 32;
        uint32_t mp[16] = {0}, mu[16] = {0};
        for (int c = 0; c < ncu; ++c) (c < panel_cus ? mp : mu)[c / 32] |= (1u << (c % 32));
        if (words <= 16 && hipExtStreamCreateWithCUMask(&la->panel, words, mp) == hipSuccess) {
            if (hipExtStreamCreateWithCUMask(&la->update, words, mu) == hipSuccess) {
                masked = true;
            } else {
                (void)hipStreamDestroy(la->panel);
// ... 56 lines not shown
                              la->ev_near[i],  la->ev_tc[i],  la->ev_tb[i],    la->ev_split[i],  la->ev_gp[i], la->ev_c1[i]};
        for (auto e : per)
            if (e) (void)hipEventDestroy(e);
    }
    for (int i = 0; i < LookAhead::kMaxTimed; ++i) {
        if (la->tu0[i]) (void)hipEventDestroy(la->tu0[i]);
        if (la->tu1[i]) (void)hipEventDestroy(la->tu1[i]);
    }
    delete la;
}

namespace {

constexpr int64_t kLeadF32Cols = 64;

bool h3_workspace_ok(const SplitWork* sw, int64_t n, int64_t kw) {
    return sw != nullptr && sw->planes != nullptr && sw->k_cap == kw && sw->rows_cap >= n + 256 && NNGP_KNOB(2) != 2;
}

int ensure_panel_split(SplitWork* sw, const float* a, int64_t ld, int64_t n, int64_t po, int64_t pw, hipStream_t s) {
    if (sw->split_panel == po) return 0;
    const int64_t ldp = 4 * sw->k_cap;
    char* col = sw->planes + (po / pw) * sw->col_stride;
    NNGP_TRY(launch_split_rows(a + (po + pw) * ld + po, ld, n - po - pw, pw, sw->scale, col + (po + pw) * ldp, ldp, s));
    sw->split_panel = po;
    return 0;
}

int lookahead_fork(LookAhead* la, hipStream_t user, hipStream_t extra = nullptr) {
    NNGP_HIP_CHECK(hipEventRecord(la->ev_in, user));
    NNGP_HIP_CHECK(hipStreamWaitEvent(la->panel, la->ev_in, 0));
    NNGP_HIP_CHECK(hipStreamWaitEvent(la->update, la->ev_in, 0));
    if (extra != nullptr) NNGP_HIP_CHECK(hipStreamWaitEvent(extra, la->ev_in, 0));
    return 0;
}

int lookahead_join(LookAhead* la, hipStream_t user) {
    NNGP_HIP_CHECK(hipEventRecord(la->ev_panel_done, la->panel));
    NNGP_HIP_CHECK(hipEventRecord(la->ev_update_done, la->update));
    NNGP_HIP_CHECK(hipStreamWaitEvent(user, la->ev_panel_done, 0));
    NNGP_HIP_CHECK(hipStreamWaitEvent(user, la->ev_update_done, 0));
    return 0;
}

int update_timer_begin(LookAhead* la, hipStream_t s) {
    if (!la->time_updates || la->tu_count >= LookAhead::kMaxTimed) return 0;
    const int t = la->tu_count;
    if (la->tu0[t] == nullptr) NNGP_HIP_CHECK(hipEventCreate(&la->tu0[t]));
    if (la->tu1[t] == nullptr) NNGP_HIP_CHECK(hipEventCreate(&la->tu1[t]));
    NNGP_HIP_CHECK(hipEventRecord(la->tu0[t], s));
    return 1;
}

int update_timer_end(LookAhead* la, hipStream_t s, double entries, double rows_cols, double kk) {
    const int t = la->tu_count++;
    NNGP_HIP_CHECK(hipEventRecord(la->tu1[t], s));
    la->tu_flops[t] = 2.0 * entries * kk;
    la->tu_bytes[t] = 8.0 * entries + 4.0 * rows_cols * kk;
    return 0;
}

double trap_entries(int64_t m, int64_t n, int64_t shift) {
    double e = 0.0;
    const int64_t full_from = (n - shift - 1 > 0) ? n - shift - 1 : 0;
    const int64_t rt = full_from < m ? full_from : m;
    e += (double)rt * (double)(shift + 1) + 0.5 * (double)rt * (double)(rt - 1);
    if (m > rt) e += (double)(m - rt) * (double)n;
    return e;
}

double region_entries(const H3RegionSpec* reg, int nreg) {
    double e = 0.0;
    for (int r = 0; r < nreg; ++r) e += trap_entries(reg[r].m, reg[r].n, reg[r].shift);
    return e;
}

double region_rows_cols(const H3RegionSpec* reg, int nreg) {
    double rc = 0.0;
    for (int r = 0; r < nreg; ++r) rc += (double)reg[r].m + (double)reg[r].n;
    return rc;
}

int h3_update_timed(LookAhead* la, float* c, int64_t ldc, const char* a, const char* b, int64_t ldp, int64_t pstride, int np, int64_t lead,
                    int64_t m, int64_t n, int64_t k, float alpha, int64_t diag_shift, SplitWork* sw, int reserve) {
    if (m <= 0 || n <= 0) return 0;
    const int timed = update_timer_begin(la, la->update);
    if (timed < 0) return timed;
    NNGP_TRY(launch_gemm_nt_h3x(c, ldc, a, b, ldp, pstride, np, lead, m, n, k, alpha, 1.0f, true, diag_shift, sw->counters, reserve,
                                la->update));
    if (timed)
        NNGP_TRY(update_timer_end(la, la->update, trap_entries(m, n, diag_shift), (double)m + (double)n,
                                  (double)np * (double)k - (double)lead));
    return 0;
}

int f32_update_trap(float* c, int64_t ld, const float* pa, const float* pb, int64_t m, int64_t n, int64_t kk, hipStream_t s) {
    if (m <= 0 || n <= 0 || kk <= 0) return 0;
    NNGP_TRY(launch_gemm_nt_f32(c, ld, pa, ld, pb, ld, n, n, kk, -1.0f, 1.0f, true, s));
    if (m > n) NNGP_TRY(launch_gemm_nt_f32(c + n * ld, ld, pa + n * ld, ld, pb, ld, m - n, n, kk, -1.0f, 1.0f, false, s));
    return 0;
}

int f32_update_below(float* c, int64_t ld, const float* p, int64_t nb2, int64_t m, int64_t wn, int64_t kk, hipStream_t s) {
    NNGP_TRY(launch_gemm_nt_f32(c + nb2 * ld, ld, p + nb2 * ld, ld, p, ld, m - nb2, nb2, kk, -1.0f, 1.0f, false, s));
    return f32_update_trap(c + nb2 * ld + nb2, ld, p + nb2 * ld, p + nb2 * ld, m - nb2, wn - nb2, kk, s);
}

int lead_pass_f32(float* a, int64_t ld, const float* lcols, const H3RegionSpec* reg, int nreg, int64_t lead, hipStream_t s) {
    for (int r = 0; r < nreg && lead > 0; ++r) {
        float* cr = a + reg[r].row0 * ld + reg[r].col0;
        const float* pa = lcols + reg[r].row0 * ld;
        const float* pb = lcols + reg[r].col0 * ld;
        if (reg[r].shift == 0) {
            NNGP_TRY(f32_update_trap(cr, ld, pa, pb, reg[r].m, reg[r].n, lead, s));
        } else {
            NNGP_TRY(launch_gemm_nt_f32(cr, ld, pa, ld, pb, ld, reg[r].m, reg[r].n, lead, -1.0f, 1.0f, false, s));
        }
    }
    return 0;
}

struct DiagSolve {
    bool h3 = false;
    const float* akk = nullptr;
    const float* dk = nullptr;
    int64_t ld = 0, w = 0;
    char* ldiag = nullptr;
    float* dfrag = nullptr;
    float* dscale = nullptr;
};

int diag_solve_begin(DiagSolve* d, bool after_first, const float* akk, int64_t ld, const float* dk, int64_t w, const SplitWork* sw, int buf,
                     hipStream_t s) {
    d->akk = akk; d->dk = dk; d->ld = ld; d->w = w;
    d->h3 = after_first && w == 1024 && sw->ldiag != nullptr && sw->dfrag != nullptr && NNGP_KNOB(2) != 5;
    if (!d->h3) return 0;
    d->ldiag = sw->ldiag + (int64_t)buf * 4 * sw->k_cap * sw->k_cap;
    d->dfrag = sw->dfrag + (int64_t)buf * sw->k_cap * 128;
    d->dscale = sw->dscale + (int64_t)buf * sw->k_cap;
    return launch_split_diag_frag(akk, ld, w, sw->scale, d->ldiag, dk, d->dfrag, d->dscale, s);
}

int diag_solve_rows(const DiagSolve& d, float* b, int64_t m, char* planes, int64_t ldp, float scale, hipStream_t s, char* planes_t = nullptr,
                    int64_t tstride = 0, int64_t row0 = 0, int64_t col0 = 0) {
    if (d.h3) return launch_trsm_panel_h3(b, d.ld, m, d.ldiag, d.dfrag, d.dscale, d.w, planes, ldp, scale, s, planes_t, tstride, row0, col0);
// ... 35 lines not shown
        double acc_area = 0.0;
        int sidx = 1;
        for (int64_t col = f0; col < n; col += nb) {
            const int64_t w = (n - col < nb) ? n - col : nb;
            acc_area += (double)(n - col) * (double)w - 0.5 * (double)w * (double)w;
            if (sidx < ns && acc_area >= total * sidx / ns) share_lo[sidx++] = col + w;
        }
        for (int i = sidx; i <= dn; ++i) share_lo[i] = n;
    }

    int take() {
        if (!active || next >= nchunks) return -1;
        const int i = next++;
        if (next >= nchunks) active = false;
        return i;
    }

    enum : int {
        kColRows = 1,
        kNextCol = 2,
        kShare = 4,
        kAll = 7
    };
    void chunk_regions(int i, int D, int64_t n, int64_t nb, int parts, H3RegionSpec* reg, int* nreg) const {
        auto width = [&](int64_t col0) { return (n - col0 < nb) ? n - col0 : nb; };
        auto add = [&](int64_t row0, int64_t col0, int64_t w, int64_t shift) {
            if (n - row0 > 0 && w > 0) reg[(*nreg)++] = H3RegionSpec{row0, col0, n - row0, w, shift};
        };
        if ((parts & kColRows) && i == 0) {
            const int64_t w0 = width(r0);
            add(r0 + w0, r0, w0, w0);
        }
        const int64_t c1 = r0 + (int64_t)(i + 1) * nb;
        if ((parts & kNextCol) && c1 < n && i + 1 < D) add(c1, c1, width(c1), 0);
        const int si = nchunks - 1 - i;
        if ((parts & kShare) && share_lo[si + 1] > share_lo[si]) add(share_lo[si], share_lo[si], share_lo[si + 1] - share_lo[si], 0);
    }
};

struct Grouped {
    float* a;
    int64_t n, ld, nb;
    LookAhead* la;
    SplitWork* sw;
    int64_t ldp;
    float ascale;
    int reserve;
    Grouped(float* a_, int64_t n_, int64_t ld_, int64_t nb_, LookAhead* la_, SplitWork* sw_)
        : a(a_), n(n_), ld(ld_), nb(nb_), la(la_), sw(sw_), ldp(4 * sw_->k_cap), ascale(-1.0f / (sw_->scale * sw_->scale)),
          reserve(NNGP_KNOB(4) > 0 ? NNGP_KNOB(4) : 32) {}
    char* plane_rows(int col, int64_t row) const { return sw->planes + (int64_t)col * sw->col_stride + row * ldp; }
    int64_t width(int64_t col0) const { return (n - col0 < nb) ? n - col0 : nb; }
    int nblk() const { return (int)((n + nb - 1) / nb); }
    int far_grid(const FarWork& far, const H3RegionSpec* reg, int nreg, int64_t lead, hipStream_t s, int helper) const {
        const char* rows = plane_rows(far.g0 + far.np - 1, 0);
        return launch_gemm_nt_h3r(a, ld, rows, rows, ldp, sw->col_stride, far.np, lead, reg, nreg, nb, ascale, 1.0f, true, sw->counters, reserve,
                                  s, nullptr, helper);
    }
    int near_update(float* c, const float* below, const char* pk_rows, int64_t nb2, int64_t m, int64_t wn, int64_t nbk, int64_t lead) const {
        NNGP_TRY(h3_update_timed(la, c + nb2 * ld, ld, pk_rows + nb2 * ldp + lead * 4, pk_rows + lead * 4, ldp, 0, 1, 0, m - nb2, wn, nbk - lead,
                                 ascale, nb2, sw, reserve));
        if (lead > 0) NNGP_TRY(f32_update_below(c, ld, below, nb2, m, wn, lead, la->update));
        return 0;
    }
};

int potrf_lookahead_grouped(float* a, int64_t n, int64_t ld, float* dinv, int32_t* clamped, float pivot_floor, LookAhead* la,
                            SplitWork* sw, hipStream_t user, int64_t nb, int D) {
    la->tu_count = 0;
    NNGP_TRY(lookahead_fork(la, user));
    const Grouped g(a, n, ld, nb, la, sw);
    const int nblk = g.nblk();
    const bool use_helper = !(NNGP_KNOB(2) >= 31 && NNGP_KNOB(2) <= 46) && g.reserve >= 8 && g.reserve % 8 == 0;
    FarWork far;
    bool wrote_t = true;

    auto far_chunk = [&](int step) -> int {
        const int i = far.take();
        if (i < 0) return 0;
        H3RegionSpec reg[4];
        int nreg = 0;
        far.chunk_regions(i, D, n, nb, FarWork::kAll, reg, &nreg);
        if (nreg == 0) return 0;
        const int64_t lead = far.g0 == 0 ? kLeadF32Cols : 0;
        const double entries = region_entries(reg, nreg);
        const int timed = update_timer_begin(la, la->update);
        if (timed < 0) return timed;
        const bool helper = use_helper && step >= 0 && entries / 65536.0 * (double)far.np >= 4.0 * 3.0 * 224.0;
        if (helper) NNGP_HIP_CHECK(hipEventRecord(la->ev_chunk[step], la->update));
        NNGP_TRY(g.far_grid(far, reg, nreg, lead, la->update, helper ? 1 : 0));
        if (helper) {
            NNGP_HIP_CHECK(hipStreamWaitEvent(la->panel, la->ev_chunk[step], 0));
            NNGP_TRY(g.far_grid(far, reg, nreg, lead, la->panel, 2));
            NNGP_HIP_CHECK(hipEventRecord(la->ev_helper[step], la->panel));
            NNGP_HIP_CHECK(hipStreamWaitEvent(la->update, la->ev_helper[step], 0));
        }
        if (timed) NNGP_TRY(update_timer_end(la, la->update, entries, region_rows_cols(reg, nreg), (double)far.np * (double)nb - (double)lead));
        return lead_pass_f32(a, ld, a, reg, nreg, lead, la->update);
    };

    int rc = 0;
    for (int k = 0; k < nblk && rc == 0; ++k) {
        const int64_t o = (int64_t)k * nb;
        const int64_t nbk = g.width(o);
        const int64_t m = n - o - nbk;
        float* akk = a + o * ld + o;
        float* dk = dinv + (o / TB) * TB * TB;
        const int g0 = (k / D) * D;
        const int gend = (g0 + D < nblk) ? g0 + D : nblk;
        if (k > 0) NNGP_HIP_CHECK(hipStreamWaitEvent(la->panel, la->ev_col[k - 1], 0));
        rc = potrf_rec(akk, nbk, ld, dk, clamped, pivot_floor, la->panel);
        NNGP_HIP_CHECK(hipEventRecord(la->ev_panel[k], la->panel));
        if (rc != 0) break;
        rc = far_chunk(k);
        if (rc != 0 || m == 0) break;
        NNGP_HIP_CHECK(hipStreamWaitEvent(la->update, la->ev_panel[k], 0));
        const int64_t nb2 = g.width(o + nbk);
        float* below = akk + nbk * ld;
        float* c = below + nbk;
        char* pk_rows = g.plane_rows(k, o + nbk);
        char* pt = (sw->planes_t != nullptr && nb == sw->k_cap && NNGP_KNOB(9) != 8) ? sw->planes_t : nullptr;
        wrote_t = wrote_t && pt != nullptr;
        rc = solve_rows_below(k > 0, akk, ld, dk, nbk, sw, below, m, pk_rows, g.ldp, sw->scale, la->update, pt, sw->col_stride, o + nbk, o);
        if (rc != 0) break;
        if (k + 1 < gend) {
            rc = launch_gemm_nt_f32(c, ld, below, ld, below, ld, nb2, nb2, nbk, -1.0f, 1.0f, true, la->update);
            NNGP_HIP_CHECK(hipEventRecord(la->ev_col[k], la->update));
            int64_t wn = (int64_t)(gend - 1 - k) * nb;
            if (wn > m) wn = m;
            if (rc == 0 && m > nb2) rc = g.near_update(c, below, pk_rows, nb2, m, wn, nbk, k == 0 ? kLeadF32Cols : 0);
        } else {
            const int np = k + 1 - g0;
            const float* rows = a + (o + nbk) * ld + (int64_t)g0 * nb;
            rc = launch_gemm_nt_f32(c, ld, rows, ld, rows, ld, nb2, nb2, (int64_t)np * nb, -1.0f, 1.0f, true, la->update);
            NNGP_HIP_CHECK(hipEventRecord(la->ev_col[k], la->update));
            far.begin(g0, np, o + nbk, (nblk - (k + 1) < D) ? nblk - (k + 1) : D, n, nb);
        }
    }
    while (rc == 0 && far.active) rc = far_chunk(-1);
    if (rc == 0) sw->l_ready = true;
    if (rc == 0 && wrote_t && sw->planes_t != nullptr) sw->lt_ready = true;
    NNGP_TRY(lookahead_join(la, user));
    return rc;
}

int potrf_lookahead_grouped_v4(float* a, int64_t n, int64_t ld, float* dinv, int32_t* clamped, float pivot_floor, LookAhead* la,
                               SplitWork* sw, hipStream_t user, int64_t nb, int D, TriInv* ti) {
    la->tu_count = 0;
    hipStream_t SP = la->panel, SU = la->update, SB = (NNGP_KNOB(8) & 2) ? la->panel : la->bulk;
#ifdef NNGP_TIMING_KNOBS
    static hipEvent_t dbg_ev[8] = {};
    const bool dbg = NNGP_KNOB(12) != 0;
    if (dbg && dbg_ev[0] == nullptr)
        for (auto& e : dbg_ev) (void)hipEventCreate(&e);
    if (dbg) (void)hipEventRecord(dbg_ev[0], user);
#endif
    NNGP_TRY(lookahead_fork(la, user, SB));
    const Grouped g(a, n, ld, nb, la, sw);
    const int nblk = g.nblk();
    const bool use_helper = (NNGP_KNOB(8) & 8) && g.reserve >= 8 && g.reserve % 8 == 0;
    const bool early_gp = (NNGP_KNOB(8) & 4) != 0;
    FarWork far;
    struct PendingHelper {
        bool on = false;
        H3RegionSpec reg[4];
        int nreg = 0, step = 0;
        int64_t lead = 0;
    } ph;

    auto far_launch = [&](const H3RegionSpec* reg, int nreg, int step, bool allow_helper) -> int {
        if (nreg == 0) return 0;
        const int64_t lead = far.g0 == 0 ? kLeadF32Cols : 0;
        const double entries = region_entries(reg, nreg);
        const bool helper = allow_helper && use_helper && lead == 0 && step >= 0 && entries / 65536.0 * (double)far.np >= 4.0 * 3.0 * 224.0;
        const int timed = update_timer_begin(la, SU);
        if (timed < 0) return timed;
        if (helper) NNGP_HIP_CHECK(hipEventRecord(la->ev_chunk[step], SU));
        NNGP_TRY(g.far_grid(far, reg, nreg, lead, SU, helper ? 1 : 0));
        if (timed) NNGP_TRY(update_timer_end(la, SU, entries, region_rows_cols(reg, nreg), (double)far.np * (double)nb - (double)lead));
        if (helper) {
            ph.on = true;
            ph.nreg = nreg;
            for (int r = 0; r < nreg; ++r) ph.reg[r] = reg[r];
            ph.step = step; ph.lead = lead;
        }
        return lead_pass_f32(a, ld, a, reg, nreg, lead, SU);
    };
    auto far_step = [&](int step, bool* colrows_event, bool* c1_event) -> int {
        const int i = far.take();
        if (i < 0) return 0;
        H3RegionSpec reg[4];
        int nreg = 0;
        far.chunk_regions(i, D, n, nb, FarWork::kColRows, reg, &nreg);
        if (nreg > 0 && step >= 0) {
            NNGP_TRY(far_launch(reg, nreg, step, false));
            NNGP_HIP_CHECK(hipEventRecord(la->ev_col[step], SU));
            *colrows_event = true;
            nreg = 0;
        }
        const bool split_c1 = (NNGP_KNOB(8) & 16) && step >= 0;
        far.chunk_regions(i, D, n, nb, FarWork::kNextCol, reg, &nreg);
        if (split_c1 && nreg > 0) {
            NNGP_TRY(far_launch(reg, nreg, step, false));
            nreg = 0;
        }
        if (split_c1) {
            NNGP_HIP_CHECK(hipEventRecord(la->ev_c1[step], SU));
            *c1_event = true;
        }
        far.chunk_regions(i, D, n, nb, FarWork::kShare, reg, &nreg);
        return far_launch(reg, nreg, step, true);
    };

    int rc = 0;
    bool side_used = false;
    const int kTriInvTail = NNGP_KNOB(10) > 0 ? NNGP_KNOB(10) : 7;
    for (int k = 0; k < nblk && rc == 0; ++k) {
        const int64_t o = (int64_t)k * nb;
        const int64_t nbk = g.width(o);
        const int64_t m = n - o - nbk;
        float* akk = a + o * ld + o;
        float* dk = dinv + (o / TB) * TB * TB;
        const int g0 = (k / D) * D;
        const int gend = (g0 + D < nblk) ? g0 + D : nblk;
        if (k > 0) NNGP_HIP_CHECK(hipStreamWaitEvent(SP, la->ev_chain[k - 1], 0));
        rc = potrf_rec(akk, nbk, ld, dk, clamped, pivot_floor, SP);
        NNGP_HIP_CHECK(hipEventRecord(la->ev_panel[k], SP));
        if (rc != 0) break;
        if (ti != nullptr && la->side != nullptr && (NNGP_KNOB(8) & 32) && k == nblk - kTriInvTail && ti->bs % nb == 0 && k >= 2) {
            const int64_t jdone = ((int64_t)(k - 1) * nb) / ti->bs;
            if (jdone > 0) {
                hipStream_t SS = NNGP_KNOB(11) == 3 ? la->aux : NNGP_KNOB(11) == 4 ? la->bulk : la->side;
// ... 280 lines not shown
```

nngp-src_amd/csrc/solve.hip:

```cpp
#include "common.h"

namespace nngp {

namespace {

__global__ __launch_bounds__(256) void k_gemv_n_f32(const float* __restrict__ A, int64_t lda, int64_t rows,
                                                    int64_t cols, const float* __restrict__ x, float* y, int sub) {
    const int lane = threadIdx.x & 63;
    const int64_t row = (int64_t)blockIdx.x * 4 + (threadIdx.x >> 6);
    if (row >= rows) return;
    const float4* ar = reinterpret_cast<const float4*>(A + row * lda);
    const float4* xv = reinterpret_cast<const float4*>(x);
    float s = 0.0f;
    for (int64_t c = lane; c < cols / 4; c += 64) {
        const float4 a = ar[c], v = xv[c];
        s = fmaf(a.x, v.x, s);
        s = fmaf(a.y, v.y, s);
        s = fmaf(a.z, v.z, s);
        s = fmaf(a.w, v.w, s);
    }
#pragma unroll
    for (int off = 32; off > 0; off >>= 1) s += __shfl_xor(s, off);
    if (lane == 0) y[row] = sub ? y[row] - s : s;
}
// ... 242 lines not shown
    NNGP_HIP_CHECK(hipGetLastError());
    return 0;
}

int triinv_build(const float* l, int64_t ld, const float* dinv, int64_t np, TriInv& ti, hipStream_t s) {
    const int64_t j0 = ti.done_blocks;
    ti.done_blocks = 0;
    return triinv_build_range(l, ld, dinv, np, ti, j0, (np + ti.bs - 1) / ti.bs, s);
}

#define kTriLower (NNGP_KNOB(9) == 4 ? 0 : 1)
#define kTriUpper (NNGP_KNOB(9) == 4 ? 0 : 2)

int trsm_rlt_blocks_f32(float* b, int64_t ldb, int64_t m, const float* l, int64_t ld, const TriInv& ti, int64_t np,
                        float* tmp, hipStream_t s) {
    const int64_t bs = ti.bs;
    for (int64_t o = 0, j = 0; o < np; o += bs, ++j) {
        const int64_t sz = (np - o < bs) ? np - o : bs;
        NNGP_TRY(launch_gemm_nt_f32(tmp, sz, b + o, ldb, ti.xinv + j * bs * bs, bs, m, sz, sz, 1.0f, 0.0f, false, s, kTriLower));
        NNGP_HIP_CHECK(hipMemcpy2DAsync(b + o, sizeof(float) * ldb, tmp, sizeof(float) * sz, sizeof(float) * sz, m,
                                        hipMemcpyDeviceToDevice, s));
        const int64_t rest = np - o - sz;
        if (rest > 0)
            NNGP_TRY(launch_gemm_nt_f32(b + o + sz, ldb, b + o, ldb, l + (o + sz) * ld + o, ld, m, rest, sz, -1.0f, 1.0f,
                                        false, s));
    }
    return 0;
}

int trsm_rut_blocks_f32(float* b, int64_t ldb, int64_t m, const float* lt, int64_t ld, const TriInv& ti, int64_t np,
                        float* tmp, hipStream_t s) {
    const int64_t bs = ti.bs;
    const int64_t nblk = (np + bs - 1) / bs;
    for (int64_t j = nblk - 1; j >= 0; --j) {
        const int64_t o = j * bs;
        const int64_t sz = (np - o < bs) ? np - o : bs;
        NNGP_TRY(launch_gemm_nt_f32(tmp, sz, b + o, ldb, ti.tinv + j * bs * bs, bs, m, sz, sz, 1.0f, 0.0f, false, s, kTriUpper));
        NNGP_HIP_CHECK(hipMemcpy2DAsync(b + o, sizeof(float) * ldb, tmp, sizeof(float) * sz, sizeof(float) * sz, m,
                                        hipMemcpyDeviceToDevice, s));
        if (o > 0)
            NNGP_TRY(launch_gemm_nt_f32(b, ldb, b + o, ldb, lt + o, ld, m, o, sz, -1.0f, 1.0f, false, s));
    }
    return 0;
}

static bool h3_worth(int64_t m, int64_t cols) { return ((m + 255) / 256) * ((cols + 255) / 256) >= 96; }

static int h3_step_update(float* c, int64_t ldc, int64_t m, int64_t n, int64_t sz, const char* wrows, const SplitWork& sw, hipStream_t s) {
    const int64_t kc = sw.k_cap, ldp = 4 * kc;
    const int np = (int)((sz + kc - 1) / kc);
    const float alpha = -1.0f / sw.scale;
    if (sz % kc == 0)
        return launch_gemm_nt_h3x(c, ldc, sw.planes_b + (int64_t)(np - 1) * sw.col_stride, wrows + (int64_t)(np - 1) * sw.col_stride, ldp,
                                  sw.col_stride, np, 0, m, n, kc, alpha, 1.0f, false, 0, sw.counters, sw.solve_reserve, s, sw.row_inv);
    for (int p = np - 1; p >= 0; --p) {
        const int64_t kp = (p == np - 1) ? sz - (int64_t)p * kc : kc;
        NNGP_TRY(launch_gemm_nt_h3(c, ldc, sw.planes_b + (int64_t)p * sw.col_stride, wrows + (int64_t)p * sw.col_stride, ldp, m, n, kp, alpha,
                                   1.0f, false, 0, sw.counters, sw.solve_reserve, s, sw.row_inv));
    }
    return 0;
}

static bool h3_step_ok(const SplitWork& sw, int64_t bs, int64_t m) {
    return bs % sw.k_cap == 0 && bs / sw.k_cap <= sw.b_panels && bs <= 2048 && m <= sw.mb_cap;
}

int trsm_rlt_blocks_h3(float* b, int64_t ldb, int64_t m, const float* l, int64_t ld, const TriInv& ti, int64_t np,
                       float* tmp, const SplitWork& sw, hipStream_t s) {
    const int64_t bs = ti.bs, kc = sw.k_cap, ldp = 4 * kc;
    NNGP_REQUIRE(sw.l_ready && h3_step_ok(sw, bs, m), "trsm_rlt_blocks_h3: split copy of L not available");
    for (int64_t o = 0, j = 0; o < np; o += bs, ++j) {
        const int64_t sz = (np - o < bs) ? np - o : bs;
        const int64_t rest = np - o - sz;
        NNGP_TRY(launch_gemm_nt_f32(tmp, sz, b + o, ldb, ti.xinv + j * bs * bs, bs, m, sz, sz, 1.0f, 0.0f, false, s, kTriLower));
        if (rest > 0 && sz == bs && h3_worth(m, rest)) {
            NNGP_TRY(launch_split_rows_rowscale(tmp, sz, m, sz, b + o, ldb, sw.planes_b, ldp, sw.row_inv, s, sw.col_stride));
            NNGP_TRY(h3_step_update(b + o + sz, ldb, m, rest, sz, sw.planes + (o / kc) * sw.col_stride + (o + sz) * ldp, sw, s));
        } else {
            NNGP_HIP_CHECK(hipMemcpy2DAsync(b + o, sizeof(float) * ldb, tmp, sizeof(float) * sz, sizeof(float) * sz, m,
                                            hipMemcpyDeviceToDevice, s));
            if (rest > 0)
                NNGP_TRY(launch_gemm_nt_f32(b + o + sz, ldb, b + o, ldb, l + (o + sz) * ld + o, ld, m, rest, sz, -1.0f, 1.0f,
                                            false, s));
        }
    }
    return 0;
}

int trsm_rut_blocks_h3(float* b, int64_t ldb, int64_t m, const float* lt, int64_t ld, const TriInv& ti, int64_t np,
                       float* tmp, const SplitWork& sw, hipStream_t s) {
    const int64_t bs = ti.bs, kc = sw.k_cap, ldp = 4 * kc;
    NNGP_REQUIRE(sw.lt_ready && h3_step_ok(sw, bs, m), "trsm_rut_blocks_h3: split copy of L^T not available");
    const int64_t nblk = (np + bs - 1) / bs;
    for (int64_t j = nblk - 1; j >= 0; --j) {
        const int64_t o = j * bs;
        const int64_t sz = (np - o < bs) ? np - o : bs;
        NNGP_TRY(launch_gemm_nt_f32(tmp, sz, b + o, ldb, ti.tinv + j * bs * bs, bs, m, sz, sz, 1.0f, 0.0f, false, s, kTriUpper));
        if (o > 0 && (lt == nullptr || (sz == bs && h3_worth(m, o)))) {
            NNGP_TRY(launch_split_rows_rowscale(tmp, sz, m, sz, b + o, ldb, sw.planes_b, ldp, sw.row_inv, s, sw.col_stride));
            NNGP_TRY(h3_step_update(b, ldb, m, o, sz, sw.planes_t + (o / kc) * sw.col_stride, sw, s));
        } else {
            NNGP_HIP_CHECK(hipMemcpy2DAsync(b + o, sizeof(float) * ldb, tmp, sizeof(float) * sz, sizeof(float) * sz, m,
                                            hipMemcpyDeviceToDevice, s));
            if (o > 0) NNGP_TRY(launch_gemm_nt_f32(b, ldb, b + o, ldb, lt + o, ld, m, o, sz, -1.0f, 1.0f, false, s));
        }
    }
    return 0;
}

int trsv_forward_f32(const float* l, int64_t ld, const TriInv& ti, int64_t np, float* b, float* x, hipStream_t s) {
    NNGP_REQUIRE(b != x, "trsv_forward: b and x must be different buffers");
// ... 161 lines not shown
```

nngp-src_amd/model.py:

```python
from __future__ import annotations

import ctypes

import numpy as np

from . import _lib
from .kernel_spec import HasSpec, KernelSpec

_GET = {"nngp": _lib.GET_NNGP, "ntk": _lib.GET_NTK}
_COV = {False: _lib.COV_NONE, None: _lib.COV_NONE, "none": _lib.COV_NONE, "diag": _lib.COV_DIAG,
        True: _lib.COV_FULL, "full": _lib.COV_FULL}


class GPModel(HasSpec):
    def __init__(self, n_cap: int, d: int, w_std, b_std, get: str = "nngp", diag_reg: float = 1e-3,
                 diag_reg_absolute_scale: bool = False, ny: int = 1, m_cap: int = 0, knobs: bool = False,
                 activations=None, input_scale=None, groups=None, group_weights=None, full_weight=1.0):
        self.spec = KernelSpec(w_std, b_std, activations, input_scale, groups, group_weights, full_weight).resolve(d)
        if get not in _GET:
            raise ValueError("get must be 'nngp' or 'ntk', got %r" % (get,))
        self.lib = _lib.load(knobs)
        self.device = _lib.require_gpu()
        self.get, self.d, self.ny, self.n_cap = get, int(d), int(ny), int(n_cap)
        self.arch = self.spec.arch()
# ... 140 lines not shown
        self.set_train(x, y)
        self.build_rows(0, self.n)
        self.factor()
        self.solve()
        return self

    def save(self, path: str):
        import torch
        if self.n == 0:
            raise _lib.NngpError("save: fit the model first")
        x, y = (t.cpu().numpy() for t in self._keep)
        info = self.info()
        np.savez(path, x=x, y=y, get=np.array(self.get), diag_reg=np.array(self._diag_reg), absolute=np.array(self._absolute),
                 n_cap=np.array(self.n_cap), alpha=self.alpha().cpu().numpy(), reg=np.array(info["reg"]),
                 **self.spec.to_fields())
        torch.cuda.synchronize()

    @classmethod
    def load(cls, path: str, m_cap: int = 0, check: bool = True):
        z = np.load(path if str(path).endswith(".npz") else str(path) + ".npz", allow_pickle=False)
        spec = KernelSpec.from_fields(z, path)
        x, y = z["x"], z["y"]
        model = cls.from_kernel_fn(spec, max(int(z["n_cap"]), x.shape[0]), x.shape[1], get=str(z["get"]), diag_reg=float(z["diag_reg"]),
                                   diag_reg_absolute_scale=bool(z["absolute"]), ny=y.shape[1], m_cap=m_cap)
        model.fit(x, y)
        if check:
            a, a0 = model.alpha().cpu().numpy(), z["alpha"]
            err = float(np.linalg.norm(a - a0) / max(np.linalg.norm(a0), 1e-300))
            if not err < 1e-8 or abs(model.info()["reg"] - float(z["reg"])) > 1e-12 * float(z["reg"]):
                raise _lib.NngpError("load: the refitted model does not reproduce the checkpoint (alpha rel. diff %.2e)" % err)
        return model

    def kernel_buffer(self, all_rows: bool = False):
        p, ld = ctypes.c_void_p(), ctypes.c_int64()
        self._check(self.lib.nngp_model_kernel_buffer(self.handle, ctypes.byref(p), ctypes.byref(ld)))
        np_cap = (self.n_cap + 127) // 128 * 128
        rows = (np_cap * np_cap) // ld.value if all_rows else self.n
        return _wrap_device(p.value, rows * ld.value, self.device, "<f8").view(rows, ld.value), ld.value

    def info(self) -> dict:
        fi = _lib.NngpFitInfo()
        self._check(self.lib.nngp_model_info(self.handle, ctypes.byref(fi)))
        return {k: getattr(fi, k) for k, _ in fi._fields_}

    def update_timer(self, enable=True):
        self._check(self.lib.nngp_model_update_timer(self.handle, 1 if enable else 0))

    def update_timer_read(self):
        n = ctypes.c_int64(0)
        ms = ctypes.c_double(0.0)
        fl = ctypes.c_double(0.0)
        self._check(self.lib.nngp_model_update_timer_read(self.handle, ctypes.byref(n), ctypes.byref(ms), ctypes.byref(fl)))
        return int(n.value), float(ms.value), float(fl.value)

    def update_timer_bytes(self):
        b = ctypes.c_double(0.0)
        self._check(self.lib.nngp_model_update_timer_bytes(self.handle, ctypes.byref(b)))
        return float(b.value)

    def residual_timer(self, enable=True):
        self._check(self.lib.nngp_model_residual_timer(self.handle, 1 if enable else 0))

    def residual_timer_read(self):
        n = ctypes.c_int64(0)
        ms, fl, ops = ctypes.c_double(0.0), ctypes.c_double(0.0), ctypes.c_double(0.0)
        self._check(self.lib.nngp_model_residual_timer_read(self.handle, ctypes.byref(n), ctypes.byref(ms), ctypes.byref(fl), ctypes.byref(ops)))
        return int(n.value), float(ms.value), float(fl.value), float(ops.value)

    def trsm_timer(self, enable=True):
        self._check(self.lib.nngp_model_trsm_timer(self.handle, 1 if enable else 0))

    def trsm_timer_read(self):
        n = ctypes.c_int64(0)
        ms, fl = ctypes.c_double(0.0), ctypes.c_double(0.0)
        self._check(self.lib.nngp_model_trsm_timer_read(self.handle, ctypes.byref(n), ctypes.byref(ms), ctypes.byref(fl)))
        return int(n.value), float(ms.value), float(fl.value)

    def residual_floor(self):
        r, d = ctypes.c_double(-1.0), ctypes.c_int32(0)
        self._check(self.lib.nngp_model_residual_floor(self.handle, ctypes.byref(r), ctypes.byref(d)))
        return float(r.value), bool(d.value)

    def alpha(self):
        import torch
        out = torch.empty((self.n, self.ny), dtype=torch.float64, device=self.device)
        self._check(self.lib.nngp_model_alpha(self.handle, _lib.ptr(out), _lib.stream_ptr()))
        return out

    def predict(self, x_test=None, cov="diag", as_numpy=True):
        import torch
        mode = _COV[cov]
        if x_test is None:
            xt, m = None, self.n
        else:
            xt = _lib.to_device_f64(x_test, self.device)
            if xt.ndim != 2 or xt.shape[1] != self.d:
                raise ValueError("x_test must be [M, %d], got %s" % (self.d, tuple(xt.shape)))
            m = int(xt.shape[0])
            xt = self._scaled(xt)
        mean = torch.empty((m, self.ny), dtype=torch.float64, device=self.device)
        out = None
        if mode == _lib.COV_DIAG:
            out = torch.empty((m,), dtype=torch.float64, device=self.device)
        elif mode == _lib.COV_FULL:
            out = torch.empty((m, m), dtype=torch.float64, device=self.device)
        if m > 0:
# ... 46 lines not shown
```

Before: 170,700 GFLOP/s.

## Split-K the tail round of h3 GEMM tiles across idle CUs with scratch reduction

Adds a tail planner for the split-f16 (h3) NT GEMM. It uses a per-tile cycle model to decide how many k-stages to split the last, partially occupied round of tiles into, per XCD. The partial sums go to a per-CU scratch area and are then reduced, so idle CUs help finish the tail instead of waiting. The scratch is wired into the Cholesky trailing updates, the far-grid updates and the solve GEMMs, and a multi-panel entry point plus per-launch shape timing are added. In exchange it costs extra scratch memory, counter resets and partial-sum reduction passes, and it relies on cost constants that may not match the hardware.

```diff
diff --git a/__graft_entry__.py b/__graft_entry__.py
--- a/__graft_entry__.py
+++ b/__graft_entry__.py
@@ -17,7 +17,7 @@
     from nngp_src_amd import _lib
     lib = _lib.load()
     assert lib.nngp_version() == 1
-    for name in _lib.ABI_SYMBOLS + _lib.GP_ABI_SYMBOLS + _lib.ACT_ABI_SYMBOLS + _lib.MLL_ABI_SYMBOLS + _lib.LOO_ABI_SYMBOLS + _lib.ARD_ABI_SYMBOLS + _lib.ADDITIVE_ABI_SYMBOLS + _lib.POOL_ABI_SYMBOLS + _lib.SPARSE_ABI_SYMBOLS + _lib.SPARSE_EVIDENCE_ABI_SYMBOLS + _lib.I8S_ABI_SYMBOLS + _lib.MATFREE_ABI_SYMBOLS:
+    for name in _lib.ABI_SYMBOLS + _lib.GP_ABI_SYMBOLS + _lib.ACT_ABI_SYMBOLS + _lib.MLL_ABI_SYMBOLS + _lib.LOO_ABI_SYMBOLS + _lib.ARD_ABI_SYMBOLS + _lib.ADDITIVE_ABI_SYMBOLS + _lib.POOL_ABI_SYMBOLS + _lib.SPARSE_ABI_SYMBOLS + _lib.SPARSE_EVIDENCE_ABI_SYMBOLS + _lib.I8S_ABI_SYMBOLS + _lib.MATFREE_ABI_SYMBOLS + _lib.H3_TAIL_ABI_SYMBOLS:
         assert hasattr(lib, name), name
 
 
diff --git a/include/nngp_h3_tail.h b/include/nngp_h3_tail.h
--- /dev/null
+++ b/include/nngp_h3_tail.h
@@ -0,0 +1,25 @@
+#ifndef NNGP_H3_TAIL_H
+#define NNGP_H3_TAIL_H
+
+#include "nngp_hip.h"
+
+#ifdef __cplusplus
+extern "C" {
+#endif
+
+int nngp_h3_tail_plan(const int32_t* regions, int32_t nreg, int32_t br, int32_t bc, int32_t lower, int32_t nstage, int32_t workers,
+                      int32_t scratch_slots, int32_t mode, int32_t* plan);
+
+int nngp_h3_tail_unit(const int32_t* regions, int32_t nreg, int32_t br, int32_t bc, int32_t lower, int32_t nstage, int32_t split,
+                      const int32_t* first, int32_t xcd, int32_t count, int32_t* unit, int32_t* limit);
+
+int nngp_gemm_nt_h3_panels(float* c, int64_t ldc, const float* a, int64_t lda, const float* b, int64_t ldb, int64_t m, int64_t n,
+                           int64_t k, int32_t npanels, int64_t lead, float alpha, float beta, float scale, int32_t lower_only, void* stream);
+
+int nngp_model_update_timer_launches(nngp_model* m, int64_t cap, double* ms, int32_t* shape, int64_t* count);
+
+#ifdef __cplusplus
+}
+#endif
+
+#endif
diff --git a/nngp-src_amd/_lib.py b/nngp-src_amd/_lib.py
--- a/nngp-src_amd/_lib.py
+++ b/nngp-src_amd/_lib.py
@@ -65,6 +65,7 @@
 I8S_ABI_SYMBOLS = ("nngp_i8s_cut_rows", "nngp_i8s_cut_sym", "nngp_i8s_residual")
 MATFREE_ABI_SYMBOLS = ("nngp_matfree_create", "nngp_matfree_destroy", "nngp_matfree_fit", "nngp_matfree_solve",
                        "nngp_matfree_predict", "nngp_matfree_alpha", "nngp_matfree_info", "nngp_kmv_f64")
+H3_TAIL_ABI_SYMBOLS = ("nngp_h3_tail_plan", "nngp_h3_tail_unit", "nngp_gemm_nt_h3_panels", "nngp_model_update_timer_launches")
 BOUND_DTC, BOUND_VFE = 0, 1
 BOUNDS = {"dtc": BOUND_DTC, "vfe": BOUND_VFE}
 
@@ -134,7 +135,19 @@
     bind_sparse_ard_prototypes(lib)
     bind_i8s_prototypes(lib)
     bind_matfree_prototypes(lib)
+    bind_h3_tail_prototypes(lib)
     _libs[knobs] = lib
+    return lib
+
+
+def bind_h3_tail_prototypes(lib):
+    vp, i64, i32, flt = ctypes.c_void_p, ctypes.c_int64, ctypes.c_int32, ctypes.c_float
+    lib.nngp_h3_tail_plan.argtypes = [vp, i32, i32, i32, i32, i32, i32, i32, i32, vp]
+    lib.nngp_h3_tail_unit.argtypes = [vp, i32, i32, i32, i32, i32, i32, vp, i32, i32, vp, ctypes.POINTER(i32)]
+    lib.nngp_gemm_nt_h3_panels.argtypes = [vp, i64, vp, i64, vp, i64, i64, i64, i64, i32, i64, flt, flt, flt, i32, vp]
+    lib.nngp_model_update_timer_launches.argtypes = [vp, i64, vp, vp, ctypes.POINTER(i64)]
+    for name in H3_TAIL_ABI_SYMBOLS:
+        getattr(lib, name).restype = ctypes.c_int
     return lib
 
 
diff --git a/nngp-src_amd/csrc/api.hip b/nngp-src_amd/csrc/api.hip
--- a/nngp-src_amd/csrc/api.hip
+++ b/nngp-src_amd/csrc/api.hip
@@ -337,6 +337,11 @@
         rc = dev_alloc(&m->split.planes, ncols * m->split.col_stride);
         if (rc == 0) rc = dev_alloc(&m->split.counters, 16);
         if (rc == 0 && hipMemset(m->split.counters, 0, 16 * sizeof(int)) != hipSuccess) rc = -1;
+        int dev = 0, cus = 0;
+        if (rc != 0 || hipGetDevice(&dev) != hipSuccess || hipDeviceGetAttribute(&cus, hipDeviceAttributeMultiprocessorCount, dev) != hipSuccess) cus = 0;
+        if (rc == 0 && cus > 0 && soft_alloc(&m->split.tail.p, h3_tail_scratch_bytes(cus)) &&
+            hipMemset(m->split.tail.p, 0, kH3TailCounterBytes) == hipSuccess)
+            m->split.tail.slots = cus;
         if (rc == 0 && !soft_alloc(&m->split.planes_t, ncols * m->split.col_stride)) m->split.planes_t = nullptr;
         if (rc == 0) rc = dev_alloc(&m->split.ldiag, 2 * kLookAheadNb * kLookAheadNb * 4);
         if (rc == 0) rc = dev_alloc(&m->split.dfrag, 2 * kLookAheadNb * 128);
@@ -691,6 +696,23 @@
     return i8s_residual_floor(m, ratio, distrusted);
 }
 
+int nngp_model_update_timer_launches(nngp_model* m, int64_t cap, double* ms, int32_t* shape, int64_t* count) {
+    NNGP_REQUIRE(m != nullptr && m->la != nullptr && count != nullptr && cap >= 0, "update_timer_launches: no timer on this model");
+    *count = m->la->tu_count;
+    if (ms == nullptr || shape == nullptr) return 0;
+    NNGP_REQUIRE(cap >= m->la->tu_count, "update_timer_launches: room for %d launches needed", m->la->tu_count);
+    for (int t = 0; t < m->la->tu_count; ++t) {
+        NNGP_HIP_CHECK(hipEventSynchronize(m->la->tu1[t]));
+        float e = 0.0f;
+        NNGP_HIP_CHECK(hipEventElapsedTime(&e, m->la->tu0[t], m->la->tu1[t]));
+        ms[t] = e;
+        const H3LaunchInfo& li = m->la->tu_info[t];
+        const int32_t row[5] = {li.tiles, li.nstage * 32, li.workers, li.split, li.last_round};
+        for (int i = 0; i < 5; ++i) shape[5 * t + i] = row[i];
+    }
+    return 0;
+}
+
 int nngp_model_update_timer_bytes(nngp_model* m, double* bytes_total) {
     NNGP_REQUIRE(m != nullptr && m->la != nullptr && bytes_total != nullptr, "update_timer_bytes: no timer on this model");
     double b = 0.0;
diff --git a/nngp-src_amd/csrc/api_ops.hip b/nngp-src_amd/csrc/api_ops.hip
--- a/nngp-src_amd/csrc/api_ops.hip
+++ b/nngp-src_amd/csrc/api_ops.hip
@@ -1,7 +1,9 @@
 #include "model.h"
 #include "gp_f64.h"
 #include "trsm_order.h"
+#include "h3_tail_plan.h"
 #include "../../include/nngp_i8s.h"
+#include "../../include/nngp_h3_tail.h"
 
 extern "C" {
 
@@ -13,6 +15,65 @@
 int nngp_trsm_ticket_queues(int32_t row_tiles, int32_t block_cols, int32_t tail_tiles, int32_t backward, int32_t workers, int32_t merged,
                             int32_t queues, int32_t* items, int32_t* queue_of, int64_t cap, int64_t* count) {
     return tk_order_export(row_tiles, block_cols, tail_tiles, backward, workers, merged, queues, items, queue_of, cap, count);
+}
+
+static int h3_tail_regions(const int32_t* regions, int32_t nreg, int32_t br, int32_t bc, int32_t lower, int32_t nstage, H3Regions* regs) {
+    NNGP_REQUIRE(regions != nullptr && nreg >= 1 && nreg <= 4 && br >= 1 && bc >= 1 && br * bc <= 256 && nstage >= 1, "h3_tail: bad launch shape");
+    *regs = H3Regions();
+    int64_t tiles = 0;
+    for (int r = 0; r < nreg; ++r) {
+        const int32_t m = regions[3 * r], n = regions[3 * r + 1], shift = regions[3 * r + 2];
+        NNGP_REQUIRE(m > 0 && n > 0 && shift >= 0 && m % 128 == 0 && n % 128 == 0 && shift % 128 == 0, "h3_tail: m, n, shift must be multiples of 128");
+        H3Region& rg = regs->r[regs->count++];
+        rg.m = m;
+        rg.n = n;
+        rg.shift = lower ? shift : 0;
+        tiles += ((int64_t)m / 256 + 1) * ((int64_t)n / 256 + 1);
+    }
+    NNGP_REQUIRE(tiles < (1 << 24), "h3_tail: too many tiles");
+    h3_count_blocks(regs, br, bc, lower != 0);
+    return 0;
+}
+
+int nngp_h3_tail_plan(const int32_t* regions, int32_t nreg, int32_t br, int32_t bc, int32_t lower, int32_t nstage, int32_t workers,
+                      int32_t scratch_slots, int32_t mode, int32_t* plan) {
+    H3Regions regs;
+    NNGP_TRY(h3_tail_regions(regions, nreg, br, bc, lower, nstage, &regs));
+    NNGP_REQUIRE(plan != nullptr && workers >= 1 && scratch_slots >= 0 && mode >= 0 && mode <= 2, "h3_tail_plan: bad argument");
+    H3TailPlan p;
+    h3_tail_plan(regs, br, bc, lower != 0, nstage, workers, scratch_slots, mode, &p);
+    const int32_t head[5] = {p.tiles, p.tail.split, p.split_tiles, p.split_slots, p.slots_per_xcd};
+    for (int i = 0; i < 5; ++i) plan[i] = head[i];
+    for (int x = 0; x < 8; ++x) {
+        plan[5 + x] = p.xcd_tiles[x];
+        plan[13 + x] = p.tail.first[x];
+    }
+    return 0;
+}
+
+int nngp_h3_tail_unit(const int32_t* regions, int32_t nreg, int32_t br, int32_t bc, int32_t lower, int32_t nstage, int32_t split,
+                      const int32_t* first, int32_t xcd, int32_t count, int32_t* unit, int32_t* limit) {
+    H3Regions regs;
+    NNGP_TRY(h3_tail_regions(regions, nreg, br, bc, lower, nstage, &regs));
+    const int slots_per_xcd = ((regs.nblk + 7) / 8) * br * bc;
+    NNGP_REQUIRE(unit != nullptr && limit != nullptr && first != nullptr && xcd >= 0 && xcd < 8 && count >= 0 && split >= 1, "h3_tail_unit: bad argument");
+    H3Tail tail = {split, {}};
+    for (int x = 0; x < 8; ++x) {
+        NNGP_REQUIRE(first[x] >= 0 && first[x] <= slots_per_xcd && (split > 1 || first[x] == slots_per_xcd), "h3_tail_unit: bad first slot");
+        tail.first[x] = first[x];
+    }
+    *limit = h3_tail_limit(tail, slots_per_xcd, xcd);
+    for (int raw = 0; raw < count; ++raw) {
+        int32_t* u = unit + 7 * raw;
+        for (int i = 0; i < 7; ++i) u[i] = 0;
+        if (raw >= *limit) continue;
+        const H3Unit w = h3_tail_unit(tail, slots_per_xcd, nstage, raw, xcd);
+        int ri = 0, bi = 0, bj = 0;
+        if (!h3_slot_tile(regs, br, bc, lower != 0, w.slot, xcd, &ri, &bi, &bj)) continue;
+        const int32_t row[7] = {1, ri, bi, bj, w.piece, w.t0, w.t1};
+        for (int i = 0; i < 7; ++i) u[i] = row[i];
+    }
+    return 0;
 }
 
 int nngp_potrf_f32(float* a, int64_t n, int64_t ld, float* dinv, int32_t* clamped, void* stream) {
@@ -155,20 +216,40 @@
 
 int nngp_gemm_nt_h3(float* c, int64_t ldc, const float* a, int64_t lda, const float* b, int64_t ldb, int64_t m, int64_t n,
                     int64_t k, float alpha, float beta, float scale, int32_t lower_only, void* stream) {
+    return nngp_gemm_nt_h3_panels(c, ldc, a, lda, b, ldb, m, n, k, 1, 0, alpha, beta, scale, lower_only, stream);
+}
+
+int nngp_gemm_nt_h3_panels(float* c, int64_t ldc, const float* a, int64_t lda, const float* b, int64_t ldb, int64_t m, int64_t n,
+                           int64_t k, int32_t npanels, int64_t lead, float alpha, float beta, float scale, int32_t lower_only, void* stream) {
     hipStream_t s = (hipStream_t)stream;
     NNGP_REQUIRE(a != nullptr && b != nullptr && c != nullptr && scale > 0.0f, "gemm_nt_h3: bad argument");
-    NNGP_REQUIRE(m > 0 && n > 0 && k > 0 && k % 32 == 0, "gemm_nt_h3: k must be a multiple of 32");
-    const int64_t mp = round_up(m, 256), np = round_up(n, 256), ldp = 4 * k;
-    char* pa = nullptr;
-    NNGP_TRY(h3_scratch_get(s, (size_t)((mp + np) * ldp + 64), &pa));
-    char* pb = pa + mp * ldp;
-    int* counters = reinterpret_cast<int*>(pb + np * ldp);
-    if (mp > m) NNGP_HIP_CHECK(hipMemsetAsync(pa + m * ldp, 0, (size_t)((mp - m) * ldp), s));
-    NNGP_HIP_CHECK(hipMemsetAsync(pb + n * ldp, 0, (size_t)((np - n) * ldp + 64), s));
-    NNGP_TRY(launch_split_rows(a, lda, m, k, scale, pa, ldp, s));
-    NNGP_TRY(launch_split_rows(b, ldb, n, k, scale, pb, ldp, s));
-    return launch_gemm_nt_h3(c, ldc, pa, pb, ldp, m, n, k, alpha / (scale * scale), beta, lower_only != 0, 0, counters,
-                             NNGP_KNOB(4) > 0 ? NNGP_KNOB(4) : 0, s);
+    NNGP_REQUIRE(m > 0 && n > 0 && k > 0 && k % 32 == 0 && npanels >= 1 && npanels <= 16, "gemm_nt_h3: k must be a multiple of 32");
+    const int64_t mp = round_up(m, 256), np = round_up(n, 256), ldp = 4 * k, pstride = (mp + np) * ldp;
+    static std::atomic<int> cus_cached{0};
+    int cus = cus_cached.load(std::memory_order_relaxed);
+    if (cus == 0) {
+        int dev = 0;
+        if (hipGetDevice(&dev) != hipSuccess || hipDeviceGetAttribute(&cus, hipDeviceAttributeMultiprocessorCount, dev) != hipSuccess || cus <= 0) cus = 256;
+        cus_cached.store(cus, std::memory_order_relaxed);
+    }
+    const int64_t tail_off = round_up(npanels * pstride + 64, 4096);
+    char* ws = nullptr;
+    NNGP_TRY(h3_scratch_get(s, (size_t)(tail_off + h3_tail_scratch_bytes(cus)), &ws));
+    int* counters = reinterpret_cast<int*>(ws + npanels * pstride);
+    const H3TailScratch tail = {ws + tail_off, cus};
+    NNGP_HIP_CHECK(hipMemsetAsync(counters, 0, 64, s));
+    NNGP_HIP_CHECK(hipMemsetAsync(tail.p, 0, kH3TailCounterBytes, s));
+    for (int j = 0; j < npanels; ++j) {
+        char* pa = ws + j * pstride;
+        char* pb = pa + mp * ldp;
+        if (mp > m) NNGP_HIP_CHECK(hipMemsetAsync(pa + m * ldp, 0, (size_t)((mp - m) * ldp), s));
+        if (np > n) NNGP_HIP_CHECK(hipMemsetAsync(pb + n * ldp, 0, (size_t)((np - n) * ldp), s));
+        NNGP_TRY(launch_split_rows(a + j * k, lda, m, k, scale, pa, ldp, s));
+        NNGP_TRY(launch_split_rows(b + j * k, ldb, n, k, scale, pb, ldp, s));
+    }
+    const char* pa = ws + (npanels - 1) * pstride;
+    return launch_gemm_nt_h3x(c, ldc, pa, pa + mp * ldp, ldp, pstride, npanels, lead, m, n, k, alpha / (scale * scale), beta, lower_only != 0, 0,
+                              counters, NNGP_KNOB(4) > 0 ? NNGP_KNOB(4) : 0, s, nullptr, &tail);
 }
 
 int nngp_gemm_nt_f64(double* c, int64_t ldc, const double* cin, int64_t ldcin, const double* a, int64_t lda,
diff --git a/nngp-src_amd/csrc/common.h b/nngp-src_amd/csrc/common.h
--- a/nngp-src_amd/csrc/common.h
+++ b/nngp-src_amd/csrc/common.h
@@ -130,18 +130,29 @@
                                char* out, int64_t out_ld, float* row_inv, hipStream_t s, int64_t pan_stride = 0);
 int launch_split_lower_t(const float* l, int64_t ld, int64_t n, int64_t bs, float scale, char* out, int64_t col_stride,
                          hipStream_t s);
+struct H3TailScratch {
+    char* p = nullptr;
+    int slots = 0;
+};
+constexpr int64_t kH3TailCounterBytes = 4096, kH3TailSlotBytes = 256 * 1024;
+inline int64_t h3_tail_scratch_bytes(int slots) { return kH3TailCounterBytes + (int64_t)slots * kH3TailSlotBytes; }
+struct H3LaunchInfo {
+    int tiles, workers, split, last_round, nstage;
+};
 int launch_gemm_nt_h3(float* c, int64_t ldc, const char* a, const char* b, int64_t ldp, int64_t m, int64_t n, int64_t k,
                       float alpha, float beta, bool lower_only, int64_t diag_shift, int* counters, int reserve_cus,
-                      hipStream_t s, const float* row_alpha = nullptr);
+                      hipStream_t s, const float* row_alpha = nullptr, const H3TailScratch* tail_ws = nullptr);
 struct H3RegionSpec {
     int64_t row0, col0, m, n, shift;
 };
 int launch_gemm_nt_h3r(float* c, int64_t ldc, const char* a, const char* b, int64_t ldp, int64_t pstride, int npanels, int64_t lead,
                        const H3RegionSpec* spec, int nreg, int64_t k, float alpha, float beta, bool lower_only, int* counters,
-                       int reserve_cus, hipStream_t s, const float* row_alpha = nullptr, int helper = 0);
+                       int reserve_cus, hipStream_t s, const float* row_alpha = nullptr, int helper = 0, const H3TailScratch* tail_ws = nullptr,
+                       H3LaunchInfo* info = nullptr);
 int launch_gemm_nt_h3x(float* c, int64_t ldc, const char* a, const char* b, int64_t ldp, int64_t pstride, int npanels, int64_t lead,
                        int64_t m, int64_t n, int64_t k, float alpha, float beta, bool lower_only, int64_t diag_shift, int* counters,
-                       int reserve_cus, hipStream_t s, const float* row_alpha = nullptr);
+                       int reserve_cus, hipStream_t s, const float* row_alpha = nullptr, const H3TailScratch* tail_ws = nullptr,
+                       H3LaunchInfo* info = nullptr);
 
 int launch_potrf_leaf(float* a, int64_t ld, float* dinv_block, int32_t* clamped, float pivot_floor, hipStream_t s);
 int potrf_f32(float* a, int64_t n, int64_t ld, float* dinv, int32_t* clamped, float pivot_floor, hipStream_t s);
@@ -166,6 +177,7 @@
     int64_t rows_cap = 0, k_cap = 0, col_stride = 0;
     float scale = 1.0f;
     int* counters = nullptr;
+    H3TailScratch tail;
     bool l_ready = false;
     int64_t split_panel = -1;
     char* ldiag = nullptr;
@@ -203,6 +215,7 @@
     int tu_count = 0;
     double tu_flops[kMaxTimed] = {};
     double tu_bytes[kMaxTimed] = {};
+    H3LaunchInfo tu_info[kMaxTimed] = {};
 };
 int lookahead_create(LookAhead** out);
 void lookahead_destroy(LookAhead* la);
diff --git a/nngp-src_amd/csrc/gemm_h3.hip b/nngp-src_amd/csrc/gemm_h3.hip
--- a/nngp-src_amd/csrc/gemm_h3.hip
+++ b/nngp-src_amd/csrc/gemm_h3.hip
@@ -1,6 +1,8 @@
+#include <algorithm>
 #include <atomic>
 
 #include "common.h"
+#include "h3_tail_plan.h"
 
 namespace nngp {
 
@@ -113,16 +115,6 @@
 
 typedef __attribute__((address_space(3))) void lds_void;
 typedef const __attribute__((address_space(1))) void glb_void;
-
-__host__ __device__ __forceinline__ int h3_block_cols(int gr, int br, int bc, int tiles_m, int tiles_n, bool lower, int sh_t) {
-    int last = tiles_n - 1;
-    if (lower) {
-        int rmax = gr * br + br - 1;
-        if (rmax > tiles_m - 1) rmax = tiles_m - 1;
-        if (rmax + sh_t < last) last = rmax + sh_t;
-    }
-    return last / bc + 1;
-}
 
 template <bool LOWER>
 __global__ __launch_bounds__(512) void k_gemm_nt_h3(float* C, int64_t ldc, const char* A, const char* B, int64_t ldp,
@@ -304,17 +296,6 @@
 
 typedef float f32x4v __attribute__((ext_vector_type(4)));
 
-struct H3Region {
-    int64_t c_off;
-    int64_t a_off;
-    int64_t b_off;
-    int m, n, shift, blk0;
-};
-struct H3Regions {
-    int count, nblk;
-    H3Region r[4];
-};
-
 #ifdef NNGP_TIMING_KNOBS
 __device__ unsigned long long g_h3_stamps[2 * 8];
 #endif
@@ -322,7 +303,8 @@
 __global__ __launch_bounds__(512) void k_gemm_nt_h3v2(float* C, int64_t ldc, const char* A, const char* B, int64_t ldp,
                                                       int64_t pstride, int npanels, int nk_first, int first_off, H3Regions regs, int nk,
                                                       float alpha, float beta, int order_br, int order_bc,
-                                                      int* counters, int slots_per_xcd, const float* row_alpha, int total_wgs) {
+                                                      int* counters, int slots_per_xcd, const float* row_alpha, int total_wgs,
+                                                      H3Tail tail, char* tail_scratch) {
     constexpr int ablate = ABL;
     __shared__ __attribute__((aligned(1024))) char smem[8 * 20480];
     int& s_slot = *reinterpret_cast<int*>(smem);
@@ -345,44 +327,34 @@
         float* pc;
         int row0, col0;
         int m, n, shift;
+        int t0, t1;
+        int piece, sid;
     };
-    auto decode = [&](int slot, Tile& tl) -> bool {
-        const int per = order_br * order_bc;
-        int G = (slot / per) * 8 + vx;
-        const int i = slot % per;
-        if (G >= regs.nblk) return false;
-        int ri = 0;
-#pragma unroll
-        for (int r = 1; r < 4; ++r)
-            if (r < regs.count && G >= regs.r[r].blk0) ri = r;
-        const int m = regs.r[ri].m, n = regs.r[ri].n, diag_shift = regs.r[ri].shift;
-        G -= regs.r[ri].blk0;
-        const int tiles_m = (m + HT - 1) / HT, tiles_n = (n + HT - 1) / HT;
-        const int brows = (tiles_m + order_br - 1) / order_br;
-        const int sh_t = (diag_shift + HT - 1) / HT;
-        int gr = 0;
-        for (; gr < brows; ++gr) {
-            const int cnt = h3_block_cols(gr, order_br, order_bc, tiles_m, tiles_n, LOWER, sh_t);
-            if (G < cnt) break;
-            G -= cnt;
-        }
-        if (gr >= brows) return false;
-        const int bi = gr * order_br + (i % order_br);
-        const int bj = G * order_bc + (i / order_br);
-        if (bi >= tiles_m || bj >= tiles_n) return false;
-        if (LOWER && bj * HT > bi * HT + HT - 1 + diag_shift) return false;
+    auto decode = [&](int raw, Tile& tl) -> bool {
+        const H3Unit u = h3_tail_unit(tail, slots_per_xcd, nstage, raw, vx);
+        int ri, bi, bj;
+        if (!h3_slot_tile(regs, order_br, order_bc, LOWER, u.slot, vx, &ri, &bi, &bj)) return false;
         tl.pa = A + regs.r[ri].a_off + (int64_t)bi * HT * ldp;
         tl.pb = B + regs.r[ri].b_off + (int64_t)bj * HT * ldp;
         tl.pc = C + regs.r[ri].c_off + (int64_t)bi * HT * ldc + (int64_t)bj * HT;
         tl.row0 = bi * HT;
         tl.col0 = bj * HT;
-        tl.m = m;
-        tl.n = n;
-        tl.shift = diag_shift;
+        tl.m = regs.r[ri].m;
+        tl.n = regs.r[ri].n;
+        tl.shift = regs.r[ri].shift;
+        tl.t0 = u.t0;
+        tl.t1 = u.t1;
+        tl.piece = u.piece;
+        tl.sid = u.sid;
         return true;
     };
+    auto slot_limit = [&]() -> int { return h3_tail_limit(tail, slots_per_xcd, vx); };
     int cur_p = 0, cur_kb = 0;
-    auto cursor_reset = [&]() { cur_p = 0; cur_kb = (npanels == 1 ? nk_first : nk) - 1; };
+    auto cursor_seek = [&](int t) {
+        cur_p = t / nk;
+        if (cur_p > npanels - 1) cur_p = npanels - 1;
+        cur_kb = (cur_p == npanels - 1 ? nk_first : nk) - 1 - (t - cur_p * nk);
+    };
     auto cursor_take = [&]() -> int64_t {
         const int64_t off = (int64_t)cur_kb * 128 - (int64_t)cur_p * pstride + (cur_p == npanels - 1 ? first_off : 0);
         if (--cur_kb < 0) {
@@ -415,7 +387,7 @@
             __syncthreads();
             const int slot = __builtin_amdgcn_readfirstlane(s_slot);
             __syncthreads();
-            if (slot >= slots_per_xcd) {
+            if (slot >= slot_limit()) {
                 if (++tries >= 8) return false;
                 vx = (vx + 1) & 7;
                 continue;
@@ -435,12 +407,13 @@
 #endif
     Tile tl = {};
     bool have = fetch_tile(tl);
-    if (have) {
-        cursor_reset();
+    auto request_first_stage = [&]() {
+        cursor_seek(tl.t0);
         const int64_t k0 = cursor_take();
         glds_b(0, k0, tl.pb);
         glds_a(0, k0, tl.pa);
-    }
+    };
+    if (have) request_first_stage();
     while (have) {
         f32x4v acc[8][4];
 #pragma unroll
@@ -453,10 +426,11 @@
         if (group == 1) __builtin_amdgcn_s_barrier();
         H3_STAMP(st_last == 0 ? -1 : 4);
         int next_slot = 0;
-        for (int t = 0; t < nstage; ++t) {
+        const int nst = tl.t1 - tl.t0;
+        for (int t = 0; t < nst; ++t) {
             const char* sa_ = smem + (t & 1) * HSTAGE;
             const char* sb_ = sa_ + HT * HROW;
-            const bool more = t + 1 < nstage && !(ablate & 1);
+            const bool more = t + 1 < nst && !(ablate & 1);
             const int64_t knext = more ? cursor_take() : 0;
             h8 bh[4], bl[4], ah[4], al[4];
 #pragma unroll
@@ -550,9 +524,10 @@
         __syncthreads();
         int slot = __builtin_amdgcn_readfirstlane(s_slot);
         __syncthreads();
-        have = slot < slots_per_xcd && decode(slot, tl);
+        const bool dry = slot >= slot_limit();
+        have = !dry && decode(slot, tl);
         if (!have) {
-            if (slot >= slots_per_xcd) {
+            if (dry) {
                 ++tries;
                 vx = (vx + 1) & 7;
             }
@@ -560,6 +535,44 @@
         }
 
         H3_STAMP(1);
+        if (ct.piece >= 0) {
+            char* part = tail_scratch + 4096 + (int64_t)ct.sid * tail.split * kH3PieceBytes;
+            const int64_t lane_part = ((int64_t)wave * 2048 + lane) * 16;
+            char* mine = part + (int64_t)ct.piece * kH3PieceBytes + lane_part;
+#pragma unroll
+            for (int i = 0; i < 8; ++i)
+#pragma unroll
+                for (int j = 0; j < 4; ++j) *reinterpret_cast<f32x4v*>(mine + (i * 4 + j) * 1024) = acc[i][j];
+            asm volatile("s_waitcnt vmcnt(0)" ::: "memory");
+            __syncthreads();
+            if (tid == 0) {
+                int* arrivals = reinterpret_cast<int*>(tail_scratch) + ct.sid;
+                __builtin_amdgcn_fence(__ATOMIC_RELEASE, "agent");
+                asm volatile("s_waitcnt vmcnt(0)" ::: "memory");
+                const int before = atomicAdd(arrivals, 1);
+                if (before == tail.split - 1) __hip_atomic_store(arrivals, 0, __ATOMIC_RELAXED, __HIP_MEMORY_SCOPE_AGENT);
+                s_slot = before;
+            }
+            __syncthreads();
+            const bool last = __builtin_amdgcn_readfirstlane(s_slot) == tail.split - 1;
+            __syncthreads();
+            if (!last) {
+                if (have) request_first_stage();
+                continue;
+            }
+            __builtin_amdgcn_fence(__ATOMIC_ACQUIRE, "agent");
+#pragma unroll 1
+            for (int p = 0; p < tail.split; ++p) {
+                const char* theirs = part + (int64_t)p * kH3PieceBytes + lane_part;
+#pragma unroll
+                for (int i = 0; i < 8; ++i)
+#pragma unroll
+                    for (int j = 0; j < 4; ++j) {
+                        const f32x4v v = *reinterpret_cast<const f32x4v*>(theirs + (i * 4 + j) * 1024);
+                        acc[i][j] = (p == 0) ? v : acc[i][j] + v;
+                    }
+            }
+        }
         const int m = ct.m, n = ct.n, diag_shift = ct.shift;
         const int row_base = ct.row0 + group * 128;
         const int col_base = ct.col0 + w4 * 64;
@@ -665,10 +678,7 @@
         if (have) {
             asm volatile("s_waitcnt lgkmcnt(0)" ::: "memory");
             __builtin_amdgcn_s_barrier();
-            cursor_reset();
-            const int64_t k0 = cursor_take();
-            glds_b(0, k0, tl.pb);
-            glds_a(0, k0, tl.pa);
+            request_first_stage();
         }
     }
 #ifdef NNGP_TIMING_KNOBS
@@ -730,7 +740,7 @@
 
 int launch_gemm_nt_h3r(float* c, int64_t ldc, const char* a, const char* b, int64_t ldp, int64_t pstride, int npanels, int64_t lead,
                        const H3RegionSpec* spec, int nreg, int64_t k, float alpha, float beta, bool lower_only, int* counters,
-                       int reserve_cus, hipStream_t s, const float* row_alpha, int helper) {
+                       int reserve_cus, hipStream_t s, const float* row_alpha, int helper, const H3TailScratch* tail_ws, H3LaunchInfo* info) {
     NNGP_REQUIRE(nreg >= 1 && nreg <= 4 && spec != nullptr, "gemm_nt_h3: 1 to 4 regions per launch");
     NNGP_REQUIRE(k > 0 && k % 32 == 0, "gemm_nt_h3: k must be a multiple of 32 (k=%lld)", (long long)k);
     NNGP_REQUIRE(ldp >= 4 * k && ldp % 16 == 0 && ((uintptr_t)a & 15) == 0 && ((uintptr_t)b & 15) == 0 && counters != nullptr,
@@ -750,7 +760,6 @@
     const int variant = (NNGP_KNOB(5) >= 10 && NNGP_KNOB(5) < 18) ? NNGP_KNOB(5) - 10 : 0;
     const int br = kOrders[variant][0], bc = kOrders[variant][1];
     H3Regions regs = {};
-    int64_t nblk = 0;
     for (int r = 0; r < nreg; ++r) {
         const H3RegionSpec& sp = spec[r];
         if (sp.m <= 0 || sp.n <= 0) continue;
@@ -764,15 +773,12 @@
         rg.m = (int)sp.m;
         rg.n = (int)sp.n;
         rg.shift = lower_only ? (int)sp.shift : 0;
-        rg.blk0 = (int)nblk;
-        const int64_t tm = (sp.m + HT - 1) / HT, tn = (sp.n + HT - 1) / HT;
-        for (int64_t gr = 0; gr < (tm + br - 1) / br; ++gr)
-            nblk += h3_block_cols((int)gr, br, bc, (int)tm, (int)tn, lower_only, (int)((rg.shift + HT - 1) / HT));
     }
     if (regs.count == 0) return 0;
-    regs.nblk = (int)nblk;
+    h3_count_blocks(&regs, br, bc, lower_only);
+    const int64_t nblk = regs.nblk;
     const int64_t slots_per_xcd = ((nblk + 7) / 8) * br * bc;
-    NNGP_REQUIRE(slots_per_xcd < 2147483647LL / 8, "gemm_nt_h3: too many tiles");
+    NNGP_REQUIRE(slots_per_xcd < 2147483647LL / 64, "gemm_nt_h3: too many tiles");
     static std::atomic<int> ncu_cached{0};
     int ncu = ncu_cached.load(std::memory_order_relaxed);
     if (ncu == 0) {
@@ -782,21 +788,30 @@
         ncu_cached.store(ncu, std::memory_order_relaxed);
     }
     int64_t grid = ncu - reserve_cus;
-    if (grid > slots_per_xcd * 8) grid = slots_per_xcd * 8;
     grid = (grid / 8) * 8;
     if (grid < 8) grid = 8;
+    if (helper != 0) NNGP_REQUIRE(form == 2 && reserve_cus >= 8 && reserve_cus % 8 == 0, "gemm_nt_h3: a helper grid needs form 2 and reserved compute units");
+    H3TailPlan plan;
+    const int nstage = (int)((npanels - 1) * (k / 32) + (k - lead) / 32);
+    const bool may_split = form == 2 && tail_ws != nullptr && tail_ws->p != nullptr;
+    h3_tail_plan(regs, br, bc, lower_only, nstage, (int)grid + (helper != 0 ? reserve_cus : 0), may_split ? tail_ws->slots : 0,
+                 !may_split || NNGP_KNOB(5) == 70 ? 1 : NNGP_KNOB(5) == 71 ? 2 : 0, &plan);
+    int64_t units = 0;
+    for (int x = 0; x < 8; ++x) units = std::max<int64_t>(units, h3_tail_limit(plan.tail, (int)slots_per_xcd, x));
+    if (grid > 8 * units) grid = 8 * units;
     int total_wgs = (int)grid;
     if (helper != 0) {
-        NNGP_REQUIRE(form == 2 && reserve_cus >= 8 && reserve_cus % 8 == 0, "gemm_nt_h3: a helper grid needs form 2 and reserved compute units");
         total_wgs = (int)grid + reserve_cus;
         if (helper == 2) grid = reserve_cus;
     }
+    if (info != nullptr) *info = H3LaunchInfo{plan.tiles, total_wgs, plan.tail.split, plan.round_tiles, nstage};
+    char* tail_scratch = may_split ? tail_ws->p : nullptr;
     const int ablate = NNGP_KNOB(0) & 507;
     if (form == 2) {
 #define NNGP_H3V2_LAUNCH(LOW, ABL)                                                                                                  \
     hipLaunchKernelGGL((k_gemm_nt_h3v2<LOW, ABL>), dim3((unsigned)grid), dim3(512), 0, s, c, ldc, a, b, ldp, pstride, npanels,          \
                        (int)((k - lead) / 32), (int)(lead * 4), regs, (int)(k / 32), alpha, beta, br, bc, counters,                  \
-                       (int)slots_per_xcd, row_alpha, total_wgs)
+                       (int)slots_per_xcd, row_alpha, total_wgs, plan.tail, tail_scratch)
 #ifdef NNGP_TIMING_KNOBS
         if (lower_only) {
             switch (ablate) {
@@ -847,19 +862,19 @@
 
 int launch_gemm_nt_h3x(float* c, int64_t ldc, const char* a, const char* b, int64_t ldp, int64_t pstride, int npanels, int64_t lead,
                        int64_t m, int64_t n, int64_t k, float alpha, float beta, bool lower_only, int64_t diag_shift, int* counters,
-                       int reserve_cus, hipStream_t s, const float* row_alpha) {
+                       int reserve_cus, hipStream_t s, const float* row_alpha, const H3TailScratch* tail_ws, H3LaunchInfo* info) {
     if (m <= 0 || n <= 0) return 0;
     NNGP_REQUIRE(ldc >= n && diag_shift % 128 == 0 && diag_shift >= 0, "gemm_nt_h3: bad ldc / diag_shift");
     const H3RegionSpec one = {0, 0, m, n, diag_shift};
     return launch_gemm_nt_h3r(c, ldc, a, b, ldp, pstride, npanels, lead, &one, 1, k, alpha, beta, lower_only, counters, reserve_cus, s,
-                              row_alpha, 0);
+                              row_alpha, 0, tail_ws, info);
 }
 
 int launch_gemm_nt_h3(float* c, int64_t ldc, const char* a, const char* b, int64_t ldp, int64_t m, int64_t n, int64_t k,
                       float alpha, float beta, bool lower_only, int64_t diag_shift, int* counters, int reserve_cus,
-                      hipStream_t s, const float* row_alpha) {
+                      hipStream_t s, const float* row_alpha, const H3TailScratch* tail_ws) {
     return launch_gemm_nt_h3x(c, ldc, a, b, ldp, 0, 1, 0, m, n, k, alpha, beta, lower_only, diag_shift, counters, reserve_cus, s,
-                              row_alpha);
-}
-
-}
+                              row_alpha, tail_ws);
+}
+
+}
diff --git a/nngp-src_amd/csrc/h3_tail_plan.cpp b/nngp-src_amd/csrc/h3_tail_plan.cpp
--- /dev/null
+++ b/nngp-src_amd/csrc/h3_tail_plan.cpp
@@ -0,0 +1,84 @@
+#include "h3_tail_plan.h"
+
+namespace nngp {
+
+double h3_tail_saving(int nstage, int s) {
+    const int longest = (nstage + s - 1) / s;
+    return kH3StageCycles * (double)(nstage - longest) - kH3PartialPassCycles * (double)(1 + s);
+}
+
+void h3_count_blocks(H3Regions* regs, int br, int bc, bool lower) {
+    int64_t nblk = 0;
+    for (int r = 0; r < regs->count; ++r) {
+        H3Region& rg = regs->r[r];
+        rg.blk0 = (int)nblk;
+        const int tm = (rg.m + kH3Tile - 1) / kH3Tile, tn = (rg.n + kH3Tile - 1) / kH3Tile;
+        for (int gr = 0; gr < (tm + br - 1) / br; ++gr) nblk += h3_block_cols(gr, br, bc, tm, tn, lower, (rg.shift + kH3Tile - 1) / kH3Tile);
+    }
+    regs->nblk = (int)nblk;
+}
+
+void h3_tail_plan(const H3Regions& regs, int br, int bc, bool lower, int nstage, int workers, int scratch_slots, int mode, H3TailPlan* out) {
+    const int per = br * bc;
+    const int slots_per_xcd = ((regs.nblk + 7) / 8) * per;
+    H3TailPlan p = {};
+    p.slots_per_xcd = slots_per_xcd;
+    p.tail.split = 1;
+    for (int x = 0; x < 8; ++x) p.tail.first[x] = slots_per_xcd;
+    int G = 0;
+    for (int r = 0; r < regs.count; ++r) {
+        const H3Region& rg = regs.r[r];
+        const int tm = (rg.m + kH3Tile - 1) / kH3Tile, tn = (rg.n + kH3Tile - 1) / kH3Tile;
+        for (int gr = 0; gr < (tm + br - 1) / br; ++gr) {
+            const int cols = h3_block_cols(gr, br, bc, tm, tn, lower, (rg.shift + kH3Tile - 1) / kH3Tile);
+            for (int gc = 0; gc < cols; ++gc, ++G)
+                for (int i = 0; i < per; ++i) {
+                    const int bi = gr * br + i % br, bj = gc * bc + i / br;
+                    if (bi < tm && bj < tn && !(lower && bj * kH3Tile > bi * kH3Tile + kH3Tile - 1 + rg.shift)) ++p.xcd_tiles[G & 7];
+                }
+        }
+    }
+    const int w = workers / 8;
+    for (int x = 0; x < 8; ++x) {
+        p.tiles += p.xcd_tiles[x];
+        p.last_round[x] = w > 0 ? p.xcd_tiles[x] % w : 0;
+    }
+    *out = p;
+    const int R = workers > 0 ? p.tiles % workers : 0;
+    p.round_tiles = R;
+    *out = p;
+    if (mode == 1 || R == 0) return;
+    int found = 0, key = 8 * slots_per_xcd;
+    while (found < R && key > 0) {
+        --key;
+        int ri, bi, bj;
+        if (h3_slot_tile(regs, br, bc, lower, key >> 3, key & 7, &ri, &bi, &bj)) ++found;
+    }
+    H3Tail tail = {2, {}};
+    for (int x = 0; x < 8; ++x) tail.first[x] = p.xcd_tiles[x] > 0 ? (key - x + 7) >> 3 : slots_per_xcd;
+    const int split_slots = h3_tail_slots(tail, slots_per_xcd);
+    int smax = workers / R;
+    if (nstage / kH3MinPieceStages < smax) smax = nstage / kH3MinPieceStages;
+    if (scratch_slots / split_slots < smax) smax = scratch_slots / split_slots;
+    if (smax < 2) return;
+    int s = smax;
+    if (mode != 2) {
+        double best = 0.0;
+        s = 1;
+        for (int c = 2; c <= smax; ++c) {
+            const double save = h3_tail_saving(nstage, c);
+            if (save > best) {
+                best = save;
+                s = c;
+            }
+        }
+        if (s == 1) return;
+    }
+    tail.split = s;
+    p.tail = tail;
+    p.split_tiles = R;
+    p.split_slots = split_slots;
+    *out = p;
+}
+
+}
diff --git a/nngp-src_amd/csrc/h3_tail_plan.h b/nngp-src_amd/csrc/h3_tail_plan.h
--- /dev/null
+++ b/nngp-src_amd/csrc/h3_tail_plan.h
@@ -0,0 +1,132 @@
+#pragma once
+#include <stdint.h>
+
+#if defined(__HIP__)
+#define NNGP_HD __attribute__((host)) __attribute__((device)) inline __attribute__((always_inline))
+#else
+#define NNGP_HD inline
+#endif
+
+namespace nngp {
+
+constexpr int kH3Tile = 256;
+constexpr int kH3MinPieceStages = 16;
+constexpr int kH3PieceBytes = 8 * 32 * 64 * 16;
+
+struct H3Region {
+    int64_t c_off;
+    int64_t a_off;
+    int64_t b_off;
+    int m, n, shift, blk0;
+};
+struct H3Regions {
+    int count, nblk;
+    H3Region r[4];
+};
+
+NNGP_HD int h3_block_cols(int gr, int br, int bc, int tiles_m, int tiles_n, bool lower, int sh_t) {
+    int last = tiles_n - 1;
+    if (lower) {
+        int rmax = gr * br + br - 1;
+        if (rmax > tiles_m - 1) rmax = tiles_m - 1;
+        if (rmax + sh_t < last) last = rmax + sh_t;
+    }
+    return last / bc + 1;
+}
+
+NNGP_HD bool h3_slot_tile(const H3Regions& regs, int br, int bc, bool lower, int slot, int x, int* ri_out, int* bi_out, int* bj_out) {
+    const int per = br * bc;
+    int G = (slot / per) * 8 + x;
+    const int i = slot % per;
+    if (G >= regs.nblk) return false;
+    int ri = 0;
+#pragma unroll
+    for (int r = 1; r < 4; ++r)
+        if (r < regs.count && G >= regs.r[r].blk0) ri = r;
+    const int m = regs.r[ri].m, n = regs.r[ri].n, diag_shift = regs.r[ri].shift;
+    G -= regs.r[ri].blk0;
+    const int tiles_m = (m + kH3Tile - 1) / kH3Tile, tiles_n = (n + kH3Tile - 1) / kH3Tile;
+    const int brows = (tiles_m + br - 1) / br;
+    const int sh_t = (diag_shift + kH3Tile - 1) / kH3Tile;
+    int gr = 0;
+    for (; gr < brows; ++gr) {
+        const int cnt = h3_block_cols(gr, br, bc, tiles_m, tiles_n, lower, sh_t);
+        if (G < cnt) break;
+        G -= cnt;
+    }
+    if (gr >= brows) return false;
+    const int bi = gr * br + (i % br);
+    const int bj = G * bc + (i / br);
+    if (bi >= tiles_m || bj >= tiles_n) return false;
+    if (lower && bj * kH3Tile > bi * kH3Tile + kH3Tile - 1 + diag_shift) return false;
+    *ri_out = ri;
+    *bi_out = bi;
+    *bj_out = bj;
+    return true;
+}
+
+struct H3Tail {
+    int split;
+    int first[8];
+};
+NNGP_HD void h3_tail_xcd(const H3Tail& tp, int slots_per_xcd, int x, int* first, int* before) {
+    int f = tp.first[0], b = 0, run = 0;
+#pragma unroll
+    for (int r = 1; r < 8; ++r) {
+        run += slots_per_xcd - tp.first[r - 1];
+        if (x == r) {
+            f = tp.first[r];
+            b = run;
+        }
+    }
+    *first = f;
+    *before = b;
+}
+NNGP_HD int h3_tail_limit(const H3Tail& tp, int slots_per_xcd, int x) {
+    if (tp.split <= 1) return slots_per_xcd;
+    int first, before;
+    h3_tail_xcd(tp, slots_per_xcd, x, &first, &before);
+    return first + (slots_per_xcd - first) * tp.split;
+}
+NNGP_HD int h3_tail_slots(const H3Tail& tp, int slots_per_xcd) {
+    int n = 0;
+#pragma unroll
+    for (int r = 0; r < 8; ++r) n += slots_per_xcd - tp.first[r];
+    return n;
+}
+struct H3Unit {
+    int slot, piece, sid, t0, t1;
+};
+NNGP_HD H3Unit h3_tail_unit(const H3Tail& tp, int slots_per_xcd, int nstage, int raw, int x) {
+    H3Unit u = {raw, -1, 0, 0, nstage};
+    if (tp.split <= 1) return u;
+    int first, before;
+    h3_tail_xcd(tp, slots_per_xcd, x, &first, &before);
+    if (raw < first) return u;
+    const int q = raw - first;
+    u.slot = first + q / tp.split;
+    u.piece = q - (u.slot - first) * tp.split;
+    u.sid = before + u.slot - first;
+    u.t0 = (int)((int64_t)u.piece * nstage / tp.split);
+    u.t1 = (int)((int64_t)(u.piece + 1) * nstage / tp.split);
+    return u;
+}
+
+struct H3TailPlan {
+    H3Tail tail;
+    int tiles;
+    int xcd_tiles[8];
+    int last_round[8];
+    int round_tiles;
+    int split_tiles;
+    int split_slots;
+    int slots_per_xcd;
+};
+constexpr double kH3TileFixedCycles = 60000.0;
+constexpr double kH3StageCycles = 3500.0;
+constexpr double kH3PartialPassCycles = 25000.0;
+double h3_tail_saving(int nstage, int s);
+void h3_tail_plan(const H3Regions& regs, int br, int bc, bool lower, int nstage, int workers, int scratch_slots, int mode, H3TailPlan* out);
+void h3_count_blocks(H3Regions* regs, int br, int bc, bool lower);
+
+}
diff --git a/nngp-src_amd/csrc/model.h b/nngp-src_amd/csrc/model.h
--- a/nngp-src_amd/csrc/model.h
+++ b/nngp-src_amd/csrc/model.h
@@ -218,7 +218,7 @@
         if (ev_lt) (void)hipEventDestroy(ev_lt);
         if (ev_tri) (void)hipEventDestroy(ev_tri);
         if (ev_tri_fork) (void)hipEventDestroy(ev_tri_fork);
-        dev_free(split.planes); dev_free(split.counters); dev_free(split.planes_t); dev_free(split.planes_b); dev_free(split.row_inv);
+        dev_free(split.planes); dev_free(split.counters); dev_free(split.tail.p); dev_free(split.planes_t); dev_free(split.planes_b); dev_free(split.row_inv);
         dev_free(split.ldiag); dev_free(split.dfrag); dev_free(split.dscale);
         tk_destroy(tk);
         dev_free(xt_q); dev_free(tt_diag); dev_free(ktd64); dev_free(b32); dev_free(trsm_tmp); dev_free(ktt64); dev_free(vvt32);
diff --git a/nngp-src_amd/csrc/potrf_lookahead.hip b/nngp-src_amd/csrc/potrf_lookahead.hip
--- a/nngp-src_amd/csrc/potrf_lookahead.hip
+++ b/nngp-src_amd/csrc/potrf_lookahead.hip
@@ -132,8 +132,9 @@
     return 1;
 }
 
-int update_timer_end(LookAhead* la, hipStream_t s, double entries, double rows_cols, double kk) {
+int update_timer_end(LookAhead* la, hipStream_t s, double entries, double rows_cols, double kk, const H3LaunchInfo& info) {
     const int t = la->tu_count++;
+    la->tu_info[t] = info;
     NNGP_HIP_CHECK(hipEventRecord(la->tu1[t], s));
     la->tu_flops[t] = 2.0 * entries * kk;
     la->tu_bytes[t] = 8.0 * entries + 4.0 * rows_cols * kk;
@@ -166,11 +167,12 @@
     if (m <= 0 || n <= 0) return 0;
     const int timed = update_timer_begin(la, la->update);
     if (timed < 0) return timed;
+    H3LaunchInfo info = {};
     NNGP_TRY(launch_gemm_nt_h3x(c, ldc, a, b, ldp, pstride, np, lead, m, n, k, alpha, 1.0f, true, diag_shift, sw->counters, reserve,
-                                la->update));
+                                la->update, nullptr, &sw->tail, &info));
     if (timed)
         NNGP_TRY(update_timer_end(la, la->update, trap_entries(m, n, diag_shift), (double)m + (double)n,
-                                  (double)np * (double)k - (double)lead));
+                                  (double)np * (double)k - (double)lead, info));
     return 0;
 }
 
@@ -312,10 +314,10 @@
     char* plane_rows(int col, int64_t row) const { return sw->planes + (int64_t)col * sw->col_stride + row * ldp; }
     int64_t width(int64_t col0) const { return (n - col0 < nb) ? n - col0 : nb; }
     int nblk() const { return (int)((n + nb - 1) / nb); }
-    int far_grid(const FarWork& far, const H3RegionSpec* reg, int nreg, int64_t lead, hipStream_t s, int helper) const {
+    int far_grid(const FarWork& far, const H3RegionSpec* reg, int nreg, int64_t lead, hipStream_t s, int helper, H3LaunchInfo* info = nullptr) const {
         const char* rows = plane_rows(far.g0 + far.np - 1, 0);
         return launch_gemm_nt_h3r(a, ld, rows, rows, ldp, sw->col_stride, far.np, lead, reg, nreg, nb, ascale, 1.0f, true, sw->counters, reserve,
-                                  s, nullptr, helper);
+                                  s, nullptr, helper, &sw->tail, info);
     }
     int near_update(float* c, const float* below, const char* pk_rows, int64_t nb2, int64_t m, int64_t wn, int64_t nbk, int64_t lead) const {
         NNGP_TRY(h3_update_timed(la, c + nb2 * ld, ld, pk_rows + nb2 * ldp + lead * 4, pk_rows + lead * 4, ldp, 0, 1, 0, m - nb2, wn, nbk - lead,
@@ -348,14 +350,15 @@
         if (timed < 0) return timed;
         const bool helper = use_helper && step >= 0 && entries / 65536.0 * (double)far.np >= 4.0 * 3.0 * 224.0;
         if (helper) NNGP_HIP_CHECK(hipEventRecord(la->ev_chunk[step], la->update));
-        NNGP_TRY(g.far_grid(far, reg, nreg, lead, la->update, helper ? 1 : 0));
+        H3LaunchInfo info = {};
+        NNGP_TRY(g.far_grid(far, reg, nreg, lead, la->update, helper ? 1 : 0, &info));
         if (helper) {
             NNGP_HIP_CHECK(hipStreamWaitEvent(la->panel, la->ev_chunk[step], 0));
             NNGP_TRY(g.far_grid(far, reg, nreg, lead, la->panel, 2));
             NNGP_HIP_CHECK(hipEventRecord(la->ev_helper[step], la->panel));
             NNGP_HIP_CHECK(hipStreamWaitEvent(la->update, la->ev_helper[step], 0));
         }
-        if (timed) NNGP_TRY(update_timer_end(la, la->update, entries, region_rows_cols(reg, nreg), (double)far.np * (double)nb - (double)lead));
+        if (timed) NNGP_TRY(update_timer_end(la, la->update, entries, region_rows_cols(reg, nreg), (double)far.np * (double)nb - (double)lead, info));
         return lead_pass_f32(a, ld, a, reg, nreg, lead, la->update);
     };
 
@@ -436,8 +439,9 @@
         const int timed = update_timer_begin(la, SU);
         if (timed < 0) return timed;
         if (helper) NNGP_HIP_CHECK(hipEventRecord(la->ev_chunk[step], SU));
-        NNGP_TRY(g.far_grid(far, reg, nreg, lead, SU, helper ? 1 : 0));
-        if (timed) NNGP_TRY(update_timer_end(la, SU, entries, region_rows_cols(reg, nreg), (double)far.np * (double)nb - (double)lead));
+        H3LaunchInfo info = {};
+        NNGP_TRY(g.far_grid(far, reg, nreg, lead, SU, helper ? 1 : 0, &info));
+        if (timed) NNGP_TRY(update_timer_end(la, SU, entries, region_rows_cols(reg, nreg), (double)far.np * (double)nb - (double)lead, info));
         if (helper) {
             ph.on = true;
             ph.nreg = nreg;
diff --git a/nngp-src_amd/csrc/solve.hip b/nngp-src_amd/csrc/solve.hip
--- a/nngp-src_amd/csrc/solve.hip
+++ b/nngp-src_amd/csrc/solve.hip
@@ -318,11 +318,11 @@
     const float alpha = -1.0f / sw.scale;
     if (sz % kc == 0)
         return launch_gemm_nt_h3x(c, ldc, sw.planes_b + (int64_t)(np - 1) * sw.col_stride, wrows + (int64_t)(np - 1) * sw.col_stride, ldp,
-                                  sw.col_stride, np, 0, m, n, kc, alpha, 1.0f, false, 0, sw.counters, sw.solve_reserve, s, sw.row_inv);
+                                  sw.col_stride, np, 0, m, n, kc, alpha, 1.0f, false, 0, sw.counters, sw.solve_reserve, s, sw.row_inv, &sw.tail);
     for (int p = np - 1; p >= 0; --p) {
         const int64_t kp = (p == np - 1) ? sz - (int64_t)p * kc : kc;
         NNGP_TRY(launch_gemm_nt_h3(c, ldc, sw.planes_b + (int64_t)p * sw.col_stride, wrows + (int64_t)p * sw.col_stride, ldp, m, n, kp, alpha,
-                                   1.0f, false, 0, sw.counters, sw.solve_reserve, s, sw.row_inv));
+                                   1.0f, false, 0, sw.counters, sw.solve_reserve, s, sw.row_inv, &sw.tail));
     }
     return 0;
 }
diff --git a/nngp-src_amd/model.py b/nngp-src_amd/model.py
--- a/nngp-src_amd/model.py
+++ b/nngp-src_amd/model.py
@@ -216,6 +216,15 @@
         fl = ctypes.c_double(0.0)
         self._check(self.lib.nngp_model_update_timer_read(self.handle, ctypes.byref(n), ctypes.byref(ms), ctypes.byref(fl)))
         return int(n.value), float(ms.value), float(fl.value)
+
+    def update_timer_launches(self):
+        n = ctypes.c_int64(0)
+        self._check(self.lib.nngp_model_update_timer_launches(self.handle, 0, None, None, ctypes.byref(n)))
+        ms = np.zeros(n.value, dtype=np.float64)
+        shape = np.zeros((n.value, 5), dtype=np.int32)
+        if n.value:
+            self._check(self.lib.nngp_model_update_timer_launches(self.handle, n.value, ms.ctypes.data, shape.ctypes.data, ctypes.byref(n)))
+        return ms, shape
 
     def update_timer_bytes(self):
         b = ctypes.c_double(0.0)
```

After: 170,100 GFLOP/s. Within noise of the previous version (-0.4%).
